# sosp2021/Reth

Measured on AMD Instinct MI355X. Metric: env-steps/sec + learner updates/sec, Ape-X DQN Pong, 1/2/4/8 MI355X, higher is better.
Workload: dtype f32

## Files before the change

include/reth_hip.h:

```cpp
#ifndef RETH_HIP_H
#define RETH_HIP_H
#include <stdint.h>

#ifdef __cplusplus
extern "C" {
#endif

#define RTH_OK 0
#define RTH_ERR_INVALID -1
#define RTH_ERR_HIP -2
#define RTH_ERR_NOMEM -3

#define RTH_U8 0
#define RTH_I32 1
#define RTH_I64 2
#define RTH_F32 3
#define RTH_F64 4
#define RTH_MAX_COLS 8
#define RTH_PRIO_RAW 16
#define RTH_FRAMES 8

const char *rth_last_error(void);
int rth_tree_update_timeouts(int64_t *out);
int rth_version(void);
// ... 182 lines not shown
                       const float *td_abs_dev, float *td_acc_dev, void *stream);
int rth_td_heads_backward(const float *q_s0_dev, const float *q_s1_online_dev, const float *q_s1_target_dev,
                          const int64_t *a_dev, const float *r_dev, const float *done_dev, const double *isw_dev,
                          int64_t B, int64_t A, float gamma_n, int32_t double_q, const float *h_dev, int64_t ldh,
                          const float *w2_dev, int32_t H2, float *td_abs_dev, float *loss_out_dev, float *gh_dev,
                          float *gw2_dev, float *gb2_dev, float *gb1_dev, float *td_acc_dev, void *stream);
int rth_heads_backward_branches(const float *dq_dev, const float *h_dev, int64_t ldh, const float *const *fc2_params_dev,
                                int32_t H, int64_t B, int64_t A, float *gh_dev, float *const *fc2_grads_dev,
                                float *gb1_dev, const float *td_abs_dev, float *td_acc_dev, void *stream);
int rth_td_heads_backward_branches(const float *q_s0_dev, const float *q_s1_online_dev, const float *q_s1_target_dev,
                                   const int64_t *a_dev, const float *r_dev, const float *done_dev,
                                   const double *isw_dev, int64_t B, int64_t A, float gamma_n, int32_t double_q,
                                   const float *h_dev, int64_t ldh, const float *const *fc2_params_dev, int32_t H,
                                   float *td_abs_dev, float *loss_out_dev, float *gh_dev,
                                   float *const *fc2_grads_dev, float *gb1_dev, float *td_acc_dev, void *stream);
int rth_heads_fc2(const float *h_dev, int64_t ldh, int64_t n, int32_t H, int32_t A, const float *const *fc2_params_dev,
                  float *heads_dev, void *stream);
int rth_heads_fc2_upto(const float *h_dev, int64_t ldh, int64_t n_max, const int64_t *n_dev, int32_t H, int32_t A,
                       const float *const *fc2_params_dev, float *heads_dev, float *cache_dev,
                       const int64_t *cache_rows_dev, void *stream);
int rth_linear_relu_rows_upto(const float *x_dev, int64_t ldx, int64_t r0, int64_t n_max, const int64_t *n_dev,
                              const float *w_dev, const float *b_dev, int64_t F, int64_t O, float *y_dev, int64_t ldy,
                              void *stream);

#define RTH_CONV_F32_NHWC 0
#define RTH_CONV_U8_CHW 1
#define RTH_CONV_OUT_NCHW 16
#define RTH_CONV_PACK_DGRAD 32
typedef struct rth_conv_shape {
  int32_t input;
  int32_t cin, hin, win, cout, kh, kw, stride;
} rth_conv_shape;
int rth_conv_supported(const rth_conv_shape *shape);
#define RTH_CONV_IMPL_F32 1
#define RTH_CONV_IMPL_BF16X3 2
#define RTH_CONV_IMPL_X9 3
int rth_conv_impl(const rth_conv_shape *shape, int64_t n, int32_t *nsamp_out);
int64_t rth_conv_packed_bytes(const rth_conv_shape *shape);
int rth_conv_pack(const rth_conv_shape *shape, const float *w_ohwi_dev, float *packed_dev, void *stream);
int rth_conv_pack_many(int32_t n, const rth_conv_shape *shapes, const float *const *w_ohwi_dev,
                       float *const *packed_dev, void *stream);
int rth_conv_bias_relu(const rth_conv_shape *shape, const void *x_dev, const int64_t *rows_dev, int64_t n,
                       const float *packed_dev, const float *bias_dev, float *y_dev, void *stream);
int rth_conv_bias_relu_upto(const rth_conv_shape *shape, const void *x_dev, const int64_t *rows_dev, int64_t n_max,
                            const int64_t *n_dev, const float *packed_dev, const float *bias_dev, float *y_dev,
                            void *stream);
int rth_conv_dgrad_supported(const rth_conv_shape *shape);
int rth_conv_dgrad(const rth_conv_shape *shape, const float *gy_dev, int64_t n, const float *w_ohwi_dev,
                   float *gx_dev, void *stream);
int64_t rth_conv_dgrad_workspace(const rth_conv_shape *shape);
int rth_conv_dgrad_prepacked(const rth_conv_shape *shape, const float *gy_dev, int64_t n, const void *packed_dev,
                             float *gx_dev, void *stream);
int rth_conv_dgrad_relu_supported(const rth_conv_shape *shape);
int rth_conv_dgrad_relu_prepacked(const rth_conv_shape *shape, const float *gy_dev, int64_t n, const void *packed_dev,
                                  const float *y_dev, float *gx_dev, void *bias_ws_dev, int64_t *slabs_out,
                                  void *stream);
int rth_conv_dgrad_relu_nchw_supported(const rth_conv_shape *shape);
int rth_conv_dgrad_relu_nchw_prepacked(const rth_conv_shape *shape, const float *g_dev, const float *y_dev, int64_t n,
                                       const void *packed_dev, const float *y_below_dev, float *gy_dev, float *gx_dev,
                                       void *bias_ws_dev, void *bias_ws_below_dev, int64_t *slabs_out, void *stream);
int rth_fc_x9_supported(int64_t M, int64_t N, int64_t K);
int64_t rth_fc_x9_workspace(int64_t M, int64_t N, int64_t K);
int rth_fc_x9(const float *x_dev, int64_t ldx, int64_t M, const float *w_dev, int64_t N, int64_t K,
              const float *bias_dev, int32_t relu, float *y_dev, void *workspace_dev, void *stream);
int rth_fc_x9_rows_upto(const float *x_dev, int64_t ldx, int64_t M, int64_t n_max, const int64_t *n_dev,
                        const float *w_dev, int64_t N, int64_t K, const float *bias_dev, float *y_dev,
                        void *workspace_dev, void *stream);
int rth_fc1_heads_supported(int64_t M, int64_t N, int64_t K, int32_t A);
int rth_fc1_heads(const float *x_dev, int64_t ldx, int64_t M, const float *w1_dev, int64_t N, int64_t K,
                  const float *b1_dev, int32_t A, const float *const *fc2_params, float *heads_dev, float *h1_out_dev,
                  void *workspace_dev, void *stream);
int rth_fc_f32_supported(int64_t M, int64_t N, int64_t K);
int64_t rth_fc_f32_workspace(int64_t M, int64_t N, int64_t K);
int rth_fc_f32(const float *x_dev, int64_t ldx, int64_t M, const float *w_dev, int64_t N, int64_t K,
               const float *bias_dev, int32_t relu, float *y_dev, void *workspace_dev, void *stream);
int rth_fc_bwd_supported(int64_t B, int64_t N, int64_t K);
int64_t rth_fc_bwd_workspace(int64_t B, int64_t N, int64_t K);
int rth_fc_bwd(const float *gy_dev, int64_t ldg, const float *x_dev, int64_t ldx, const float *w_dev, int64_t B,
               int64_t N, int64_t K, float *gx_dev, float *gw_dev, void *workspace_dev, void *stream);
int rth_conv_dgrad_ws(const rth_conv_shape *shape, const float *gy_dev, int64_t n, const float *w_ohwi_dev,
                      float *gx_dev, void *workspace_dev, void *stream);
int rth_conv_wgrad_x9_supported(const rth_conv_shape *shape);
int64_t rth_conv_wgrad_x9_workspace(const rth_conv_shape *shape);
int rth_conv_wgrad_x9(const rth_conv_shape *shape, const float *x_dev, int64_t n, const float *gy_dev, float *gw_dev,
                      void *workspace_dev, void *stream);
int rth_conv_wgrad_f32_supported(const rth_conv_shape *shape);
int64_t rth_conv_wgrad_f32_workspace(const rth_conv_shape *shape);
int rth_conv_wgrad_f32(const rth_conv_shape *shape, const float *x_dev, int64_t n, const float *gy_dev, float *gw_dev,
                       void *workspace_dev, void *stream);
typedef struct rth_wgrad_deferred {
  const float *partial;
  float *gw;
  int32_t splits, elems, nb, K;
} rth_wgrad_deferred;
int rth_conv_wgrad_f32_partials(const rth_conv_shape *shape, const float *x_dev, int64_t n, const float *gy_dev,
                                float *gw_dev, void *workspace_dev, rth_wgrad_deferred *job_out, void *stream);
int64_t rth_conv_wgrad_workspace(const rth_conv_shape *shape);
int rth_conv_relu_wgrad(const rth_conv_shape *shape, const void *x_dev, const int64_t *rows_dev, int64_t n,
                        const float *g_dev, const float *y_dev, float *gw_dev, float *gb_dev, void *workspace_dev,
                        void *stream);
typedef struct rth_bias_deferred {
  const void *workspace;
  float *db;
  int64_t rows;
  int32_t C;
  int32_t slabs;
} rth_bias_deferred;
int rth_conv_relu_wgrad_ex(const rth_conv_shape *shape, const void *x_dev, const int64_t *rows_dev, int64_t n,
                           const float *g_dev, const float *y_dev, float *gw_dev, float *gb_dev, void *workspace_dev,
                           const rth_bias_deferred *deferred, int32_t ndeferred,
                           const rth_wgrad_deferred *wdeferred, int32_t nwdeferred, void *stream);
int rth_conv1_frames_bias_relu(const rth_conv_shape *shape, const uint8_t *store_dev, const int32_t *ids_dev,
                               int64_t n, const float *packed_dev, const float *bias_dev, float *y_dev, void *stream);
int rth_conv1_frames_relu_wgrad_ex(const rth_conv_shape *shape, const uint8_t *store_dev, const int32_t *ids_dev,
                                   int64_t n, const float *g_dev, const float *y_dev, float *gw_dev, float *gb_dev,
                                   void *workspace_dev, const rth_bias_deferred *deferred, int32_t ndeferred,
                                   const rth_wgrad_deferred *wdeferred, int32_t nwdeferred, void *stream);

typedef struct rth_atari rth_atari;
int rth_atari_create(int32_t in_h, int32_t in_w, int32_t out_h, int32_t out_w, int device, rth_atari **out);
int rth_atari_destroy(rth_atari *h);
int rth_atari_step(rth_atari *h, const uint8_t *raw_dev, int64_t n, uint8_t *frames_dev, int32_t ring, int32_t stack,
                   const int64_t *prev_slot_dev, const int64_t *new_slot_dev, const uint8_t *reset_dev,
                   uint8_t *out_frame_dev, void *stream);
int rth_atari_env_step(rth_atari *h, const uint8_t *raw_dev, int64_t n, uint8_t *frames_dev, int32_t ring,
                       int32_t stack, const int64_t *s0_h_dev, const int64_t *s1_h_dev, const float *done_dev,
                       const int64_t *cur_slot_dev, const uint8_t *reset_raw_dev, void *stream);
int rth_atari_synth_raw(uint8_t *raw_dev, int64_t nbytes, uint64_t seed, const int64_t *t_dev, void *stream);
int rth_atari_synth_reset(uint8_t *reset_raw_dev, int64_t n, int64_t frame_bytes, uint64_t seed, const int64_t *t_dev,
                          const float *done_dev, void *stream);

#define RTH_MAX_PARAM_TENSORS 32
typedef struct rth_param_tensor {
  float *param;
  const float *grad;
  float *exp_avg;
  float *exp_avg_sq;
  int64_t n;
} rth_param_tensor;
int64_t rth_clip_adam_workspace(void);
int rth_clip_adam(const rth_param_tensor *tensors, int32_t n_tensors, double lr, double beta1, double beta2,
                  double eps, double max_norm, int64_t *step_dev, void *workspace_dev, float *total_norm_out_dev,
                  void *stream);
int rth_conv1_relu_wgrad_norm(const rth_conv_shape *shape, const void *x_dev, const int64_t *rows_dev,
                              const int32_t *fids_dev, int64_t n, const float *g_dev, const float *y_dev,
                              float *gw_dev, float *gb_dev, void *workspace_dev, const rth_bias_deferred *deferred,
                              int32_t ndeferred, const rth_wgrad_deferred *wdeferred, int32_t nwdeferred,
                              const rth_param_tensor *sq, int32_t n_sq, double lr, double beta1,
                              double beta2, int64_t *step_dev, void *adam_workspace_dev, int32_t *nparts_out,
                              void *stream);
int rth_adam_prenormed(const rth_param_tensor *tensors, int32_t n_tensors, double lr, double beta1, double beta2,
                       double eps, double max_norm, int32_t nparts, int64_t *step_dev, void *workspace_dev,
                       float *total_norm_out_dev, void *stream);

int rth_mlp_supported(int64_t D, int64_t H, int64_t A);
int64_t rth_mlp_workspace(int64_t B, int64_t D, int64_t H, int64_t A);
int rth_mlp_q(const float *const *params, const float *x_dev, int64_t ldx, int64_t n, int64_t D, int64_t H, int64_t A,
              float *q_dev, int32_t *argmax_dev, void *stream);
int rth_mlp_dqn_grads(const float *const *online, const float *const *target, const float *s0_dev, int64_t lds0,
                      const float *s1_dev, int64_t lds1, const int64_t *a_dev, const float *r_dev,
                      const float *done_dev, const double *isw_dev, int64_t B, int64_t D, int64_t H, int64_t A,
                      float gamma_n, int32_t double_q, float *const *grads, float *td_abs_dev, float *loss_dev,
                      void *workspace_dev, void *stream);

typedef struct rth_mlp_actor_args {
  const float *const *params;
  int64_t D, H, A;
  double *state;
  int32_t *ep_steps;
  int64_t *t_dev;
  int64_t *stats;
  float *obs_ring;
  int64_t *cur_slot;
  const double *eps;
  const int64_t *action_in;
  int64_t *action;
  float *reward, *done;
  int64_t *s0_h, *s1_h;
  int32_t *emit;
  int64_t *row_s0, *row_a, *row_s1;
  float *row_r, *row_done;
  float *row_obs0, *row_obs1;
  float *q_out;
  uint64_t seed;
  int64_t N;
  int32_t ring;
  int32_t max_episode_steps;
} rth_mlp_actor_args;
int rth_cartpole_reset(const rth_mlp_actor_args *args, void *stream);
int rth_mlp_actor_step(rth_nstep *h, const rth_mlp_actor_args *args, void *stream);

enum { RTH_ENV_CARTPOLE = 0, RTH_ENV_ACROBOT = 1, RTH_ENV_MOUNTAINCAR = 2 };
typedef struct rth_env_actor_args {
  const float *const *params;
  int64_t env;
  int64_t D, H, A;
  double *state;
  int32_t *ep_steps;
  int64_t *t_dev;
  int64_t *stats;
  double *ret_stats;
  float *obs_ring;
  int64_t *cur_slot;
  const double *eps;
  const int64_t *action_in;
  int64_t *action;
  float *reward, *done;
  int64_t *s0_h, *s1_h;
  int32_t *emit;
  int64_t *row_s0, *row_a, *row_s1;
  float *row_r, *row_done;
  float *row_obs0, *row_obs1;
  float *q_out;
  uint64_t seed;
  int64_t N;
  int32_t ring;
  int32_t max_episode_steps;
} rth_env_actor_args;
int rth_env_reset(const rth_env_actor_args *args, void *stream);
int rth_env_actor_step(rth_nstep *h, const rth_env_actor_args *args, void *stream);

int rth_ddpg_supported(int64_t D, int64_t Ad, int64_t H1, int64_t H2);
int64_t rth_ddpg_workspace(int64_t B, int64_t D, int64_t Ad, int64_t H1, int64_t H2);
int rth_ddpg_act(const float *const *actor, const float *x_dev, int64_t ldx, int64_t n, int64_t D, int64_t Ad,
                 int64_t H1, int64_t H2, float *act_out_dev, void *stream);
int rth_ddpg_critic_grads(const float *const *critic, const float *const *actor_target,
                          const float *const *critic_target, const float *s0_dev, int64_t lds0, const float *a_dev,
                          int64_t lda, const float *r_dev, const float *done_dev, const float *s1_dev, int64_t lds1,
                          const float *isw_dev, int64_t B, int64_t D, int64_t Ad, int64_t H1, int64_t H2, float gamma,
                          float *const *grads, float *td_abs_dev, float *loss_dev, void *workspace_dev, void *stream);
int rth_ddpg_actor_grads(const float *const *actor, const float *const *critic, const float *s0_dev, int64_t lds0,
                         int64_t B, int64_t D, int64_t Ad, int64_t H1, int64_t H2, float *const *grads,
                         float *loss_dev, void *workspace_dev, void *stream);
int rth_soft_update(float *const *target, const float *const *source, const int64_t *numel, int32_t n_tensors,
                    double tau, void *stream);

int rth_ppo_supported(int64_t D, int64_t H, int64_t A);
int64_t rth_ppo_workspace(int64_t B, int64_t D, int64_t H, int64_t A);
int rth_ppo_act(const float *const *actor, const float *x_dev, int64_t ldx, int64_t n, int64_t D, int64_t H, int64_t A,
                const double *uniforms_dev, uint64_t seed, uint64_t counter, int64_t *action_dev, float *logprob_dev,
                float *probs_dev, void *stream);
int rth_ppo_grads(const float *const *actor, const float *const *value, const float *s_dev, int64_t lds,
                  const int64_t *a_dev, const float *ret_dev, const float *old_logprob_dev, int64_t B, int64_t D,
                  int64_t H, int64_t A, float eps_clip, float vf_coef, float ent_coef, float *const *actor_grads,
                  float *const *value_grads, float *loss_abs_dev, float *loss_mean_dev, void *workspace_dev,
                  void *stream);
int rth_ppo_grads_n(const float *const *actor, const float *const *value, const float *s_dev, int64_t lds,
                    const int64_t *a_dev, const float *ret_dev, const float *old_logprob_dev, int64_t B, int64_t D,
                    int64_t H, int64_t A, float eps_clip, float vf_coef, float ent_coef, float *const *actor_grads,
                    float *const *value_grads, float *loss_abs_dev, float *loss_mean_dev, void *workspace_dev,
                    const int64_t *n_dev, void *stream);
int rth_ppo_grads_adv(const float *const *actor, const float *const *value, const float *s_dev, int64_t lds,
                      const int64_t *a_dev, const float *ret_dev, const float *adv_dev, const float *old_logprob_dev,
                      int64_t B, int64_t D, int64_t H, int64_t A, float eps_clip, float vf_coef, float ent_coef,
                      float *const *actor_grads, float *const *value_grads, float *loss_abs_dev, float *loss_mean_dev,
                      void *workspace_dev, const int64_t *n_dev, void *stream);
int rth_ppo_adv_normalize(float *adv_dev, int64_t B, const int64_t *n_dev, void *stream);
int64_t rth_ppo_shuffle_workspace(int64_t B);
int rth_ppo_shuffle(const float *s_dev, int64_t lds, const int64_t *a_dev, const float *ret_dev, const float *adv_dev,
                    const float *old_logprob_dev, int64_t B, const int64_t *n_dev, int64_t D, int64_t K, uint64_t seed,
                    int64_t *counter_dev, const uint64_t *keys_in, float *mb_s_dev, int64_t *mb_a_dev,
                    float *mb_ret_dev, float *mb_adv_dev, float *mb_logprob_dev, int64_t *mb_n_dev, int32_t *perm_dev,
                    void *workspace_dev, void *stream);

typedef struct rth_ppo_actor_args {
  const float *const *actor;
  int64_t env;
  int64_t D, H, A;
  double *state;
  int32_t *ep_steps;
  int64_t *t_dev;
  int64_t *stats;
  double *ret_stats;
  float *cur_obs;
  const int64_t *action_in;
  const double *uniforms_in;
  int64_t *action;
  float *logprob;
  float *seg_s;
  int64_t *seg_a;
  float *seg_r, *seg_done, *seg_logp;
  int32_t *fill;
  int32_t *complete;
  int32_t *gen;
  int64_t *dropped;
  uint64_t seed;
  int64_t N;
  int32_t cap;
  int32_t max_episode_steps;
} rth_ppo_actor_args;
int rth_ppo_env_reset(const rth_ppo_actor_args *args, void *stream);
int rth_ppo_actor_step(const rth_ppo_actor_args *args, void *stream);
int rth_ppo_rollout_finish(const rth_ppo_actor_args *args, double gamma, float *batch_s_dev, int64_t *batch_a_dev,
                           float *batch_ret_dev, float *batch_logprob_dev, int64_t *n_dev, void *stream);
int rth_ppo_gae_finish(const rth_ppo_actor_args *args, const float *const *value, double gamma, double lam,
                       float *batch_s_dev, int64_t *batch_a_dev, float *batch_ret_dev, float *batch_adv_dev,
                       float *batch_v_dev, float *batch_logprob_dev, int64_t *n_dev, void *stream);
int rth_ppo_actor_step_tl(const rth_ppo_actor_args *args, float *seg_trunc_dev, float *seg_term_s_dev, void *stream);
int rth_ppo_gae_finish_tl(const rth_ppo_actor_args *args, const float *const *value, double gamma, double lam,
                          float *batch_s_dev, int64_t *batch_a_dev, float *batch_ret_dev, float *batch_adv_dev,
                          float *batch_v_dev, float *batch_logprob_dev, int64_t *n_dev, const float *seg_trunc_dev,
                          const float *seg_term_s_dev, void *stream);

enum { RTH_DDPG_ENV_PENDULUM = 0 };
typedef struct rth_ddpg_actor_args {
  const float *const *actor;
// ... 46 lines not shown
```

reth_amd/_lib.py:

```python
import ctypes
import os

_HERE = os.path.dirname(os.path.abspath(__file__))
LIB_PATH = os.environ.get("RTH_LIB_PATH") or os.path.join(_HERE, "libreth_hip.so")

RTH_U8, RTH_I32, RTH_I64, RTH_F32, RTH_F64 = 0, 1, 2, 3, 4
RTH_PRIO_RAW = 16
RTH_FRAMES = 8
SAMPLER_PER, SAMPLER_UNIFORM, SAMPLER_FIFO = 0, 1, 2
MAX_COLS = 8

c_i32, c_i64, c_u64, c_f32, c_f64, c_vp = (ctypes.c_int32, ctypes.c_int64, ctypes.c_uint64,
                                          ctypes.c_float, ctypes.c_double, ctypes.c_void_p)


class HipExtensionMissing(ImportError):
    pass


class RethHipError(RuntimeError):
    pass


class ColDesc(ctypes.Structure):
# ... 79 lines not shown
                ("cap", c_i32), ("max_episode_steps", c_i32)]


DDPG_ENV_PENDULUM = 0


class DdpgActorArgs(ctypes.Structure):
    _fields_ = [("actor", ctypes.POINTER(c_vp)), ("env", c_i64), ("D", c_i64), ("Ad", c_i64), ("H1", c_i64),
                ("H2", c_i64), ("state", c_vp), ("ep_steps", c_vp), ("t_dev", c_vp), ("stats", c_vp),
                ("ret_stats", c_vp), ("noise", c_vp), ("cur_obs", c_vp), ("action_in", c_vp), ("act_det", c_vp),
                ("row_s0", c_vp), ("row_a", c_vp), ("row_r", c_vp), ("row_s1", c_vp), ("row_done", c_vp),
                ("seed", c_u64), ("N", c_i64), ("mu", c_f64), ("theta", c_f64), ("sigma", c_f64),
                ("eps_start", c_f64), ("eps_end", c_f64), ("eps_steps", c_i64), ("max_episode_steps", c_i32),
                ("reserved", c_i32)]


SIGNATURES = {
    "rth_last_error": (ctypes.c_char_p, []),
    "rth_version": (c_i32, []),
    "rth_build_id": (ctypes.c_char_p, []),
    "rth_graph_upload": (c_i32, [c_vp, c_vp]),
    "rth_stream_capture_deps": (c_i32, [c_vp]),
    "rth_sumtree_create": (c_i32, [c_i64, c_i32, ctypes.POINTER(c_vp)]),
    "rth_sumtree_destroy": (c_i32, [c_vp]),
    "rth_sumtree_clear": (c_i32, [c_vp, c_vp]),
    "rth_sumtree_update": (c_i32, [c_vp, c_vp, c_vp, c_i64, c_vp]),
    "rth_sumtree_find": (c_i32, [c_vp, c_vp, c_i64, c_vp, c_vp, c_vp]),
    "rth_sumtree_sample": (c_i32, [c_vp, c_i64, c_vp, c_u64, c_u64, c_vp, c_vp, c_vp]),
    "rth_sumtree_stats": (c_i32, [c_vp, c_vp, c_vp]),
    "rth_sumtree_export": (c_i32, [c_vp, c_vp, c_vp, c_vp, c_vp]),
    "rth_sumtree_import": (c_i32, [c_vp, c_vp, c_vp, c_vp, c_vp]),
    "rth_sumtree_capacity": (c_i64, [c_vp]),
    "rth_per_normalize": (c_i32, [c_vp, c_i64, c_f32, c_vp, c_vp]),
    "rth_per_update": (c_i32, [c_vp, c_vp, c_vp, c_i32, c_i64, c_f64, c_vp]),
    "rth_per_sample": (c_i32, [c_vp, c_i64, c_f64, c_vp, c_u64, c_u64, c_vp, c_vp, c_vp]),
    "rth_replay_create": (c_i32, [c_i64, c_i32, ctypes.POINTER(ColDesc), c_i32, ctypes.POINTER(Sched),
                                  ctypes.POINTER(Sched), c_i32, c_u64, ctypes.POINTER(c_vp)]),
    "rth_replay_destroy": (c_i32, [c_vp]),
    "rth_replay_append": (c_i32, [c_vp, ctypes.POINTER(Src), c_vp, c_i32, c_i64, c_vp, c_vp]),
    "rth_replay_sample": (c_i32, [c_vp, c_i64, c_vp, ctypes.POINTER(c_vp), c_vp, c_vp, c_vp]),
    "rth_replay_update_priorities": (c_i32, [c_vp, c_vp, c_vp, c_i32, c_i64, c_i32, c_vp]),
    "rth_replay_update_priorities_deferred": (c_i32, [c_vp, c_vp, c_vp, c_i32, c_i64, c_i32, c_vp]),
    "rth_replay_flush": (c_i32, [c_vp, c_vp]),
    "rth_replay_gather": (c_i32, [c_vp, c_vp, c_i64, ctypes.POINTER(c_vp), c_vp]),
    "rth_replay_info": (c_i32, [c_vp, ctypes.POINTER(c_i64), ctypes.POINTER(c_i64),
                                ctypes.POINTER(c_i64), ctypes.POINTER(c_i64), ctypes.POINTER(c_i64),
                                ctypes.POINTER(c_i64)]),
    "rth_uniform_indices": (c_i32, [c_i64, c_i64, c_vp, c_u64, c_u64, c_vp, c_vp, c_vp]),
    "rth_replay_tree": (c_vp, [c_vp]),
    "rth_replay_set_timing": (c_i32, [c_vp, ctypes.POINTER(c_vp), c_i32, ctypes.POINTER(c_i32)]),
    "rth_replay_column": (c_vp, [c_vp, c_i32]),
    "rth_replay_frames_attach": (c_i32, [c_vp, c_i64, c_i64, ctypes.POINTER(c_vp), ctypes.POINTER(c_vp)]),
    "rth_replay_push_frames": (c_i32, [c_vp, c_vp, c_i64, c_i32, c_i32, c_vp, c_vp, c_vp, c_vp, c_vp, c_i32, c_vp]),
    "rth_replay_frames_ids_out": (c_i32, [c_vp, c_i32]),
    "rth_copy_rows": (c_i32, [c_vp, c_i64, c_vp, c_vp, c_i64, c_vp, c_i64, c_i64, c_i32, c_i32, c_i32, c_vp]),
    "rth_eps_greedy": (c_i32, [c_vp, c_i64, c_i64, c_i32, c_vp, c_vp, c_vp, c_u64, c_u64, c_vp, c_vp, c_vp]),
    "rth_counter_add": (c_i32, [c_vp, c_i64, c_vp]),
    "rth_actor_prologue": (c_i32, [c_vp, c_vp, c_i64, c_i64, c_vp, c_vp]),
    "rth_compact_flagged": (c_i32, [c_vp, c_vp, c_i64, c_vp, c_i64, c_i64, c_i64, c_vp, c_vp]),
    "rth_actor_tail": (c_i32, [c_vp, ctypes.POINTER(ActorTailArgs), c_vp, c_vp, c_vp, c_vp, c_vp, c_vp, c_vp]),
    "rth_nstep_create": (c_i32, [c_i64, c_i32, c_f64, c_i32, c_i32, ctypes.POINTER(c_vp)]),
    "rth_nstep_destroy": (c_i32, [c_vp]),
    "rth_nstep_reset": (c_i32, [c_vp, c_vp]),
    "rth_nstep_push": (c_i32, [c_vp] + [c_vp] * 11 + [c_vp]),
    "rth_synth_env_step": (c_i32, [c_vp, c_i64, c_i32, c_i64, c_vp, c_vp, c_vp, c_u64, c_f32, c_f32,
                                   c_vp, c_vp, c_vp, c_vp, c_vp]),
    "rth_synth_env_reset": (c_i32, [c_vp, c_i64, c_i32, c_u64, c_vp, c_vp]),
    "rth_game_reset": (c_i32, [ctypes.POINTER(GameArgs), c_vp, c_i64, c_i32, c_vp, c_vp]),
    "rth_game_env_step": (c_i32, [ctypes.POINTER(GameArgs), c_vp, c_i64, c_i32, c_i64, c_vp, c_vp, c_vp, c_vp, c_vp,
                                  c_vp, c_vp, c_vp]),
    "rth_game_actor_tail": (c_i32, [c_vp, ctypes.POINTER(ActorTailArgs), ctypes.POINTER(GameArgs), c_vp, c_vp, c_vp,
                                    c_vp, c_vp, c_vp, c_vp]),
    "rth_td_huber": (c_i32, [c_vp] * 7 + [c_i64, c_i64, c_f32, c_i32, c_i32] + [c_vp] * 5 + [c_vp]),
    "rth_bias_relu": (c_i32, [c_vp, c_vp, c_i64, c_i32, c_vp]),
    "rth_relu_bias_grad_workspace": (c_i64, [c_i32]),
    "rth_heads_merge": (c_i32, [ctypes.POINTER(c_vp), c_i64, c_i64, c_i64, c_i32, c_i32, c_vp, c_vp, c_vp, c_vp,
                                c_vp]),
    "rth_heads_split_grad": (c_i32, [c_vp, c_vp, c_vp, c_vp, c_i64, c_i64, c_i64, c_i32, c_i32,
                                     ctypes.POINTER(c_vp), c_vp]),
    "rth_heads_backward": (c_i32, [c_vp, c_vp, c_i64, c_vp, c_i64, c_i32, c_i32, c_vp, c_vp, c_vp, c_vp, c_vp, c_vp,
                                   c_vp]),
    "rth_td_heads_backward": (c_i32, [c_vp, c_vp, c_vp, c_vp, c_vp, c_vp, c_vp, c_i64, c_i64, c_f32, c_i32, c_vp,
                                      c_i64, c_vp, c_i32, c_vp, c_vp, c_vp, c_vp, c_vp, c_vp, c_vp, c_vp]),
    "rth_heads_backward_branches": (c_i32, [c_vp, c_vp, c_i64, ctypes.POINTER(c_vp), c_i32, c_i64, c_i64, c_vp,
                                            ctypes.POINTER(c_vp), c_vp, c_vp, c_vp, c_vp]),
    "rth_td_heads_backward_branches": (c_i32, [c_vp, c_vp, c_vp, c_vp, c_vp, c_vp, c_vp, c_i64, c_i64, c_f32, c_i32,
                                               c_vp, c_i64, ctypes.POINTER(c_vp), c_i32, c_vp, c_vp, c_vp,
                                               ctypes.POINTER(c_vp), c_vp, c_vp, c_vp]),
    "rth_heads_fc2": (c_i32, [c_vp, c_i64, c_i64, c_i32, c_i32, ctypes.POINTER(c_vp), c_vp, c_vp]),
    "rth_heads_fc2_upto": (c_i32, [c_vp, c_i64, c_i64, c_vp, c_i32, c_i32, ctypes.POINTER(c_vp), c_vp, c_vp, c_vp,
                                   c_vp]),
    "rth_linear_relu_rows_upto": (c_i32, [c_vp, c_i64, c_i64, c_i64, c_vp, c_vp, c_vp, c_i64, c_i64, c_vp, c_i64,
                                          c_vp]),
    "rth_conv_wgrad_x9_supported": (c_i32, [ctypes.POINTER(ConvShape)]),
    "rth_conv_wgrad_x9_workspace": (c_i64, [ctypes.POINTER(ConvShape)]),
    "rth_conv_wgrad_x9": (c_i32, [ctypes.POINTER(ConvShape), c_vp, c_i64, c_vp, c_vp, c_vp, c_vp]),
    "rth_conv_wgrad_f32_supported": (c_i32, [ctypes.POINTER(ConvShape)]),
    "rth_conv_wgrad_f32_workspace": (c_i64, [ctypes.POINTER(ConvShape)]),
    "rth_conv_wgrad_f32": (c_i32, [ctypes.POINTER(ConvShape), c_vp, c_i64, c_vp, c_vp, c_vp, c_vp]),
    "rth_conv_wgrad_f32_partials": (c_i32, [ctypes.POINTER(ConvShape), c_vp, c_i64, c_vp, c_vp, c_vp,
                                            ctypes.POINTER(WgradDeferred), c_vp]),
    "rth_relu_bias_grad": (c_i32, [c_vp, c_vp, c_vp, c_vp, c_vp, c_i64, c_i32, c_vp]),
    "rth_relu_bias_grad_nchw": (c_i32, [c_vp, c_vp, c_vp, c_vp, c_vp, c_i64, c_i32, c_i32, c_vp]),
    "rth_conv_supported": (c_i32, [ctypes.POINTER(ConvShape)]),
    "rth_conv_packed_bytes": (c_i64, [ctypes.POINTER(ConvShape)]),
    "rth_conv_impl": (c_i32, [ctypes.POINTER(ConvShape), c_i64, c_vp]),
    "rth_conv_pack": (c_i32, [ctypes.POINTER(ConvShape), c_vp, c_vp, c_vp]),
    "rth_conv_wgrad_workspace": (c_i64, [ctypes.POINTER(ConvShape)]),
    "rth_conv_relu_wgrad": (c_i32, [ctypes.POINTER(ConvShape), c_vp, c_vp, c_i64, c_vp, c_vp, c_vp, c_vp, c_vp,
                                    c_vp]),
    "rth_conv_relu_wgrad_ex": (c_i32, [ctypes.POINTER(ConvShape), c_vp, c_vp, c_i64, c_vp, c_vp, c_vp, c_vp, c_vp,
                                       c_vp, c_i32, c_vp, c_i32, c_vp]),
    "rth_conv1_frames_relu_wgrad_ex": (c_i32, [ctypes.POINTER(ConvShape), c_vp, c_vp, c_i64, c_vp, c_vp, c_vp, c_vp,
                                               c_vp, c_vp, c_i32, c_vp, c_i32, c_vp]),
    "rth_conv_pack_many": (c_i32, [c_i32, ctypes.POINTER(ConvShape), ctypes.POINTER(c_vp), ctypes.POINTER(c_vp),
                                   c_vp]),
    "rth_conv_bias_relu": (c_i32, [ctypes.POINTER(ConvShape), c_vp, c_vp, c_i64, c_vp, c_vp, c_vp, c_vp]),
    "rth_conv1_frames_bias_relu": (c_i32, [ctypes.POINTER(ConvShape), c_vp, c_vp, c_i64, c_vp, c_vp, c_vp, c_vp]),
    "rth_conv_bias_relu_upto": (c_i32, [ctypes.POINTER(ConvShape), c_vp, c_vp, c_i64, c_vp, c_vp, c_vp, c_vp, c_vp]),
    "rth_conv_dgrad_supported": (c_i32, [ctypes.POINTER(ConvShape)]),
    "rth_conv_dgrad": (c_i32, [ctypes.POINTER(ConvShape), c_vp, c_i64, c_vp, c_vp, c_vp]),
    "rth_conv_dgrad_workspace": (c_i64, [ctypes.POINTER(ConvShape)]),
    "rth_fc_x9_supported": (c_i32, [c_i64, c_i64, c_i64]),
    "rth_fc_x9_workspace": (c_i64, [c_i64, c_i64, c_i64]),
    "rth_fc_x9": (c_i32, [c_vp, c_i64, c_i64, c_vp, c_i64, c_i64, c_vp, c_i32, c_vp, c_vp, c_vp]),
    "rth_fc_x9_rows_upto": (c_i32, [c_vp, c_i64, c_i64, c_i64, c_vp, c_vp, c_i64, c_i64, c_vp, c_vp, c_vp, c_vp]),
    "rth_fc1_heads_supported": (c_i32, [c_i64, c_i64, c_i64, c_i32]),
    "rth_fc1_heads": (c_i32, [c_vp, c_i64, c_i64, c_vp, c_i64, c_i64, c_vp, c_i32, ctypes.POINTER(c_vp), c_vp, c_vp,
                              c_vp, c_vp]),
    "rth_fc_f32_supported": (c_i32, [c_i64, c_i64, c_i64]),
    "rth_fc_f32_workspace": (c_i64, [c_i64, c_i64, c_i64]),
    "rth_fc_f32": (c_i32, [c_vp, c_i64, c_i64, c_vp, c_i64, c_i64, c_vp, c_i32, c_vp, c_vp, c_vp]),
    "rth_fc_bwd_supported": (c_i32, [c_i64, c_i64, c_i64]),
    "rth_fc_bwd_workspace": (c_i64, [c_i64, c_i64, c_i64]),
    "rth_fc_bwd": (c_i32, [c_vp, c_i64, c_vp, c_i64, c_vp, c_i64, c_i64, c_i64, c_vp, c_vp, c_vp, c_vp]),
    "rth_conv_dgrad_ws": (c_i32, [ctypes.POINTER(ConvShape), c_vp, c_i64, c_vp, c_vp, c_vp, c_vp]),
    "rth_conv_dgrad_prepacked": (c_i32, [ctypes.POINTER(ConvShape), c_vp, c_i64, c_vp, c_vp, c_vp]),
    "rth_conv_dgrad_relu_supported": (c_i32, [ctypes.POINTER(ConvShape)]),
    "rth_conv_dgrad_relu_prepacked": (c_i32, [ctypes.POINTER(ConvShape), c_vp, c_i64, c_vp, c_vp, c_vp, c_vp,
                                              ctypes.POINTER(c_i64), c_vp]),
    "rth_conv_dgrad_relu_nchw_supported": (c_i32, [ctypes.POINTER(ConvShape)]),
    "rth_conv_dgrad_relu_nchw_prepacked": (c_i32, [ctypes.POINTER(ConvShape), c_vp, c_vp, c_i64, c_vp, c_vp, c_vp, c_vp,
                                                   c_vp, c_vp, ctypes.POINTER(c_i64), c_vp]),
    "rth_atari_create": (c_i32, [c_i32, c_i32, c_i32, c_i32, c_i32, ctypes.POINTER(c_vp)]),
    "rth_atari_destroy": (c_i32, [c_vp]),
    "rth_atari_step": (c_i32, [c_vp, c_vp, c_i64, c_vp, c_i32, c_i32, c_vp, c_vp, c_vp, c_vp, c_vp]),
    "rth_atari_env_step": (c_i32, [c_vp, c_vp, c_i64, c_vp, c_i32, c_i32, c_vp, c_vp, c_vp, c_vp, c_vp, c_vp]),
    "rth_atari_synth_raw": (c_i32, [c_vp, c_i64, c_u64, c_vp, c_vp]),
    "rth_atari_synth_reset": (c_i32, [c_vp, c_i64, c_i64, c_u64, c_vp, c_vp, c_vp]),
    "rth_clip_adam_workspace": (c_i64, []),
    "rth_tree_update_timeouts": (c_i32, [ctypes.POINTER(c_i64)]),
    "rth_clip_adam": (c_i32, [c_vp, c_i32, c_f64, c_f64, c_f64, c_f64, c_f64, c_vp, c_vp, c_vp, c_vp]),
    "rth_adam_prenormed": (c_i32, [c_vp, c_i32, c_f64, c_f64, c_f64, c_f64, c_f64, c_i32, c_vp, c_vp, c_vp, c_vp]),
    "rth_conv1_relu_wgrad_norm": (c_i32, [ctypes.POINTER(ConvShape), c_vp, c_vp, c_vp, c_i64, c_vp, c_vp, c_vp, c_vp,
                                          c_vp, c_vp, c_i32, c_vp, c_i32, c_vp, c_i32, c_f64, c_f64, c_f64, c_vp, c_vp,
                                          ctypes.POINTER(c_i32), c_vp]),
    "rth_mlp_supported": (c_i32, [c_i64, c_i64, c_i64]),
    "rth_mlp_workspace": (c_i64, [c_i64, c_i64, c_i64, c_i64]),
    "rth_mlp_q": (c_i32, [ctypes.POINTER(c_vp), c_vp, c_i64, c_i64, c_i64, c_i64, c_i64, c_vp, c_vp, c_vp]),
    "rth_mlp_dqn_grads": (c_i32, [ctypes.POINTER(c_vp), ctypes.POINTER(c_vp), c_vp, c_i64, c_vp, c_i64, c_vp, c_vp,
                                  c_vp, c_vp, c_i64, c_i64, c_i64, c_i64, c_f32, c_i32, ctypes.POINTER(c_vp), c_vp,
                                  c_vp, c_vp, c_vp]),
    "rth_ddpg_supported": (c_i32, [c_i64, c_i64, c_i64, c_i64]),
    "rth_ddpg_workspace": (c_i64, [c_i64, c_i64, c_i64, c_i64, c_i64]),
    "rth_ddpg_act": (c_i32, [ctypes.POINTER(c_vp), c_vp, c_i64, c_i64, c_i64, c_i64, c_i64, c_i64, c_vp, c_vp]),
    "rth_ddpg_critic_grads": (c_i32, [ctypes.POINTER(c_vp), ctypes.POINTER(c_vp), ctypes.POINTER(c_vp), c_vp, c_i64,
                                      c_vp, c_i64, c_vp, c_vp, c_vp, c_i64, c_vp, c_i64, c_i64, c_i64, c_i64, c_i64,
                                      c_f32, ctypes.POINTER(c_vp), c_vp, c_vp, c_vp, c_vp]),
    "rth_ddpg_actor_grads": (c_i32, [ctypes.POINTER(c_vp), ctypes.POINTER(c_vp), c_vp, c_i64, c_i64, c_i64, c_i64,
                                     c_i64, c_i64, ctypes.POINTER(c_vp), c_vp, c_vp, c_vp]),
    "rth_soft_update": (c_i32, [ctypes.POINTER(c_vp), ctypes.POINTER(c_vp), ctypes.POINTER(c_i64), c_i32, c_f64,
                                c_vp]),
    "rth_ppo_supported": (c_i32, [c_i64, c_i64, c_i64]),
    "rth_ppo_workspace": (c_i64, [c_i64, c_i64, c_i64, c_i64]),
    "rth_ppo_act": (c_i32, [ctypes.POINTER(c_vp), c_vp, c_i64, c_i64, c_i64, c_i64, c_i64, c_vp, c_u64, c_u64, c_vp,
                            c_vp, c_vp, c_vp]),
    "rth_ppo_grads": (c_i32, [ctypes.POINTER(c_vp), ctypes.POINTER(c_vp), c_vp, c_i64, c_vp, c_vp, c_vp, c_i64, c_i64,
                              c_i64, c_i64, c_f32, c_f32, c_f32, ctypes.POINTER(c_vp), ctypes.POINTER(c_vp), c_vp, c_vp,
                              c_vp, c_vp]),
    "rth_ppo_grads_n": (c_i32, [ctypes.POINTER(c_vp), ctypes.POINTER(c_vp), c_vp, c_i64, c_vp, c_vp, c_vp, c_i64,
                                c_i64, c_i64, c_i64, c_f32, c_f32, c_f32, ctypes.POINTER(c_vp), ctypes.POINTER(c_vp),
                                c_vp, c_vp, c_vp, c_vp, c_vp]),
    "rth_ppo_grads_adv": (c_i32, [ctypes.POINTER(c_vp), ctypes.POINTER(c_vp), c_vp, c_i64, c_vp, c_vp, c_vp, c_vp,
                                  c_i64, c_i64, c_i64, c_i64, c_f32, c_f32, c_f32, ctypes.POINTER(c_vp),
                                  ctypes.POINTER(c_vp), c_vp, c_vp, c_vp, c_vp, c_vp]),
    "rth_ppo_adv_normalize": (c_i32, [c_vp, c_i64, c_vp, c_vp]),
    "rth_ppo_shuffle_workspace": (c_i64, [c_i64]),
    "rth_ppo_shuffle": (c_i32, [c_vp, c_i64, c_vp, c_vp, c_vp, c_vp, c_i64, c_vp, c_i64, c_i64, c_u64, c_vp, c_vp, c_vp,
                                c_vp, c_vp, c_vp, c_vp, c_vp, c_vp, c_vp, c_vp]),
    "rth_ppo_gae_finish": (c_i32, [ctypes.POINTER(PpoActorArgs), ctypes.POINTER(c_vp), c_f64, c_f64, c_vp, c_vp, c_vp,
                                   c_vp, c_vp, c_vp, c_vp, c_vp]),
    "rth_ppo_env_reset": (c_i32, [ctypes.POINTER(PpoActorArgs), c_vp]),
    "rth_ppo_actor_step": (c_i32, [ctypes.POINTER(PpoActorArgs), c_vp]),
    "rth_ppo_actor_step_tl": (c_i32, [ctypes.POINTER(PpoActorArgs), c_vp, c_vp, c_vp]),
    "rth_ppo_gae_finish_tl": (c_i32, [ctypes.POINTER(PpoActorArgs), ctypes.POINTER(c_vp), c_f64, c_f64, c_vp, c_vp, c_vp,
                                      c_vp, c_vp, c_vp, c_vp, c_vp, c_vp, c_vp]),
    "rth_ppo_rollout_finish": (c_i32, [ctypes.POINTER(PpoActorArgs), c_f64, c_vp, c_vp, c_vp, c_vp, c_vp, c_vp]),
    "rth_cartpole_reset": (c_i32, [ctypes.POINTER(MlpActorArgs), c_vp]),
    "rth_mlp_actor_step": (c_i32, [c_vp, ctypes.POINTER(MlpActorArgs), c_vp]),
    "rth_env_reset": (c_i32, [ctypes.POINTER(EnvActorArgs), c_vp]),
    "rth_env_actor_step": (c_i32, [c_vp, ctypes.POINTER(EnvActorArgs), c_vp]),
    "rth_ddpg_env_reset": (c_i32, [ctypes.POINTER(DdpgActorArgs), c_vp]),
    "rth_ddpg_actor_step": (c_i32, [ctypes.POINTER(DdpgActorArgs), c_vp]),
    "rth_weights_create": (c_i32, [c_i64, c_i32, ctypes.POINTER(c_vp)]),
    "rth_weights_destroy": (c_i32, [c_vp]),
    "rth_weights_bytes": (c_i64, [c_vp]),
    "rth_weights_publish": (c_i32, [c_vp, c_i32, ctypes.POINTER(c_vp), ctypes.POINTER(c_i64), c_vp]),
    "rth_weights_fill": (c_i32, [c_vp, c_i32, ctypes.POINTER(c_vp), ctypes.POINTER(c_i64), c_vp]),
    "rth_weights_acquire": (c_i32, [c_vp, c_i32, ctypes.POINTER(c_vp), ctypes.POINTER(c_i64), c_vp, c_vp, c_vp, c_i64,
                                    c_vp, c_vp]),
    "rth_weights_version": (c_i32, [c_vp, ctypes.POINTER(c_i64)]),
    "rth_weights_version_ptr": (c_i32, [c_vp, ctypes.POINTER(c_vp)]),
    "rth_lz4_frame_bound": (c_i32, [c_vp, c_i64, ctypes.POINTER(c_i64)]),
    "rth_lz4_frame_decompress": (c_i32, [c_vp, c_i64, c_vp, c_i64, ctypes.POINTER(c_i64)]),
    "rth_lz4_frame_compress_bound": (c_i64, [c_i64]),
    "rth_lz4_frame_compress": (c_i32, [c_vp, c_i64, c_vp, c_i64, ctypes.POINTER(c_i64)]),
    "rth_xxh32": (ctypes.c_uint32, [c_vp, c_i64, ctypes.c_uint32]),
}

_lib = None
_load_error = None

_SRC_EXT = (".hip", ".hpp", ".cpp", ".h")
HIPCC_FLAGS = ["--offload-arch=gfx950", "-O3", "-fPIC", "-shared", "-std=c++17", "-Wall",
               "-Xclang", "-target-feature", "-Xclang", "-packed-fp32-ops"]


def source_files(root=None):
    root = root or os.path.dirname(_HERE)
    csrc = os.path.join(root, "reth_amd", "csrc")
    rel = sorted(f"reth_amd/csrc/{f}" for f in os.listdir(csrc) if f.endswith(_SRC_EXT))
    return rel + ["include/reth_hip.h"]


def source_build_id(root=None):
    import hashlib

    root = root or os.path.dirname(_HERE)
    h = hashlib.sha1()
    h.update((" ".join(HIPCC_FLAGS) + "\n").encode())
    for rel in source_files(root):
        with open(os.path.join(root, rel), "rb") as f:
            data = f.read()
        blob = hashlib.sha1(b"blob %d\0" % len(data) + data).hexdigest()
        h.update(f"{blob} {rel}\n".encode())
    return h.hexdigest()


def library_build_id(path=None):
    import re

    path = path or LIB_PATH
    try:
        with open(path, "rb") as f:
            m = re.search(rb"RTH_BUILD_ID:([0-9a-f]{40})", f.read())
    except OSError:
        return None
    return m.group(1).decode() if m else None


def _load():
    global _lib, _load_error
    if _lib is not None:
        return _lib
    if not os.path.exists(LIB_PATH):
        _load_error = f"{LIB_PATH} not built (run __graft_entry__.build())"
        raise HipExtensionMissing(_load_error)
    try:
        lib = ctypes.CDLL(LIB_PATH)
    except OSError as e:
        _load_error = str(e)
        raise HipExtensionMissing(f"cannot load {LIB_PATH}: {e}") from e
    for name, (res, args) in SIGNATURES.items():
        fn = getattr(lib, name)
        fn.restype = res
        fn.argtypes = args
    _lib = lib
    return lib


def lib():
    return _load()


def check(rc, what=""):
    if rc != 0:
        msg = _load().rth_last_error().decode(errors="replace")
        raise RethHipError(f"{what or 'libreth_hip'} failed ({rc}): {msg}")


def call(name, *args):
    rc = getattr(_load(), name)(*args)
    check(rc, name)
    return rc


def ptr(t):
    if t is None:
        return None
    return t.data_ptr()


def stream_ptr(stream=None):
    import torch

    s = stream if stream is not None else torch.cuda.current_stream()
# ... 7 lines not shown
```

reth_amd/apex.py:

```python
from dataclasses import dataclass, field
from typing import Optional

import torch

from .actors import OBS_SHAPE, VecActors, apex_columns
from .dist import GradAllReduce
from .model import DQNNetwork
from .replay import HbmReplay
from .reth_buffer import TorchCudaLoader, _SERVICES, start_per
from .solver import Box, DQNSolver, Discrete
from .trainer import Trainer
from .weights import WeightsSlot, WeightsSubscriber

_CAPTURE_MODE = "thread_local"


def _end_part(parts, stream):
    import warnings

    from . import _lib

    empty = _lib.lib().rth_stream_capture_deps(stream.cuda_stream) == 0
    if not empty:
        parts[-1].capture_end()
# ... 113 lines not shown
        return cfg.capacity + reset + (cfg.n_step + 16) * cfg.n_actors + 16

    def close(self):
        _SERVICES.pop(self.addr, None)
        self._graphs = None
        if self.cfg.tuned_gemm:
            from . import gemm_tuning

            gemm_tuning.restore()

    @torch.no_grad()
    def greedy_eval(self, n_envs=256, seed=12345, eps=0.0, action_fn=None):
        cfg = self.cfg
        if cfg.env != "paddle":
            raise RuntimeError("greedy_eval plays the paddle env (ApexConfig.env = 'paddle')")
        torch.cuda.synchronize(self.device)
        net = getattr(self, "_eval_net", None)
        if net is None:
            fmt = torch.channels_last if cfg.channels_last else torch.contiguous_format
            net = self._eval_net = DQNNetwork(OBS_SHAPE, cfg.num_actions).to(self.device, memory_format=fmt)
            net.requires_grad_(False)
            net.hwc_features = bool(cfg.channels_last)
            net.hip_conv = bool(cfg.hip_conv)
        for dst, src in zip(net.parameters(), self.solver.q_network.parameters()):
            dst.copy_(src)
        net.freeze_heads()
        ev = VecActors(n_envs, cfg.num_actions, cfg.n_step, cfg.gamma, self.device, seed=seed, eps=eps,
                       channels_last=cfg.channels_last, env="paddle", balls_per_episode=cfg.balls_per_episode)
        first = torch.zeros(ev.N, dtype=torch.int64, device=self.device)
        got = torch.zeros(ev.N, dtype=torch.bool, device=self.device)
        episodes, _, last, _ = ev.episode_stats()
        for _ in range(38 * cfg.balls_per_episode):
            if action_fn is not None:
                ev.action_in = action_fn(ev)
            ev.step(net)
            new = (episodes > 0) & ~got
            first = torch.where(new, last, first)
            got |= new
        return float((first.sum() / got.sum().clamp(min=1)).item())

    @torch.no_grad()
    def prefill(self, n_rows, chunk=16384):
        g = torch.Generator(device=self.device)
        g.manual_seed(self.cfg.seed + 17 * self.rank)
        done = 0
        if self.replay.frames is not None:
            return self._prefill_frames(n_rows, g, chunk)
        while done < n_rows:
            m = min(chunk, n_rows - done)
            s0 = torch.randint(0, 256, (m, *OBS_SHAPE), dtype=torch.uint8, device=self.device, generator=g)
            s1 = torch.randint(0, 256, (m, *OBS_SHAPE), dtype=torch.uint8, device=self.device, generator=g)
            a = torch.randint(0, self.cfg.num_actions, (m,), dtype=torch.int64, device=self.device, generator=g)
            r = (torch.rand(m, device=self.device, generator=g) < self.cfg.p_reward).float()
            d = (torch.rand(m, device=self.device, generator=g) < self.cfg.p_done).float()
            td = 1.0 - torch.rand(m, device=self.device, generator=g)
            self.replay.append([s0, a, r, s1, d], td)
            done += m

    @torch.no_grad()
    def _prefill_frames(self, n_rows, g, chunk):
        store, K = self.replay.frames, OBS_SHAPE[0]
        F = store.shape[0]
        base = int(self.replay.frame_head)
        nf = n_rows + 2 * K - 1
        if base + nf > F:
            raise ValueError(f"prefill of {n_rows} rows needs {nf} frames behind {base}, the store holds {F}")
        for f0 in range(0, nf, chunk):
            m = min(chunk, nf - f0)
            store[base + f0:base + f0 + m] = torch.randint(0, 256, (m, *store.shape[1:]), dtype=torch.uint8,
                                                           device=self.device, generator=g)
        self.replay.frame_head.fill_(base + nf)
        done = 0
        while done < n_rows:
            m = min(chunk, n_rows - done)
            j = torch.arange(base + done, base + done + m, dtype=torch.int32, device=self.device)[:, None]
            ks = torch.arange(K, dtype=torch.int32, device=self.device)[None, :]
            s0, s1 = (j + ks).contiguous(), (j + K - 1 + ks).contiguous()
            a = torch.randint(0, self.cfg.num_actions, (m,), dtype=torch.int64, device=self.device, generator=g)
            r = (torch.rand(m, device=self.device, generator=g) < self.cfg.p_reward).float()
            d = (torch.rand(m, device=self.device, generator=g) < self.cfg.p_done).float()
            td = 1.0 - torch.rand(m, device=self.device, generator=g)
            self.replay.append([s0, a, r, s1, d], td)
            done += m
        if self.actors.pushes:
            raise RuntimeError("prefill a frame-store replay before the actors step")
        self.actors.attach_frame_store(self.replay)

    def _actor_compute(self):
        if self.cfg.fused_actor:
            return self.actors.step_fused(self.actor_net)
        if self.actors.step(self.actor_net):
            return self.actors.prioritise(self.actor_net), None
        return None, None

    def _learner_train(self, slot):
        data, idx, isw = slot
        return self.trainer.train(data, weights=isw)

    def _actor_host(self):
        if self.subscriber.maybe_load(self.actor_net, self.actors.t):
            self.actors.weights_changed()
            self._ev_acquired = torch.cuda.Event()
            self._ev_acquired.record()

    def _learner_host(self):
        self.trainer.account()
        self.updates += 1
        if self.solver._update_target_interval is not None and not self.solver.auto_target_update:
            self.solver._update_target_interval()
        if self.updates % self.cfg.send_weights_interval == 0:
            if self._ev_acquired is not None:
                torch.cuda.current_stream(self.device).wait_event(self._ev_acquired)
            self.slot.publish(self.solver.q_network)

    def iteration(self):
        if not hasattr(self, "_stream"):
            self._stream = torch.cuda.Stream(self.device, priority=self.cfg.extra.get("actor_priority", 0))
            self._stream.wait_stream(torch.cuda.current_stream(self.device))
        with torch.cuda.stream(self._stream):
            self._iteration()

    def _iteration(self):
        if self._graphs is None and self.cfg.hip_graph and self._graph_ready():
            self._capture()
        if self._graphs is not None:
            return self._iteration_graph()
        for _ in range(self.cfg.actor_steps_per_update):
            self._actor_host()
            td, rows = self._actor_compute()
            if td is not None:
                self.actors.append(self.replay, td, rows)
            self.env_steps += self.actors.N
        if not self.svc.ready():
            return
        if not self.loader.pending():
            self.loader.issue()
        slot = self.loader.take()
        td = self._learner_train(slot)
        self.loader.issue()
        self.replay.update_priorities(slot[1], td, step=True, deferred=True)
        self._learner_host()

    def _graph_ready(self):
        return self.actors.warm and self.updates >= 2 and self.loader.pending() == 1

    def _capture(self):
        solver = self.solver
        solver.auto_target_update = False
        slots = self.loader._slots
        tun = torch.cuda.tunable
        tuning = tun.is_enabled() and tun.tuning_is_enabled()
        if tuning:
            tun.tuning_enable(False)
        try:
            self._capture_graphs(solver, slots)
        finally:
            if tuning:
                tun.tuning_enable(True)

    def _capture_graphs(self, solver, slots):
        host = (self.actors.t, self.actors.pushes)
        side = torch.cuda.Stream(self.device)
        side.wait_stream(torch.cuda.current_stream(self.device))
        split = solver.grad_hook is not None
        G = dict(act=[], act_out=[], tgt=[], q1t=[], learn={}, learn_td={}, buckets={}, grads={})
        psets = [False, True] if self.cfg.extra.get("probe_conv2") else [False]
        with torch.cuda.stream(side):
            act = self.actors
            fresh = act.fresh
            modes = ["full"] + (["dedup"] if self.cfg.fused_actor and self.actor_net.hip_torso else [])
            G["act"], G["act_out"] = {}, {}
            for pr in psets:
                for mode in modes:
                    for _ in range(2):
                        k = act.pushes % 2
                        act.fresh = act.n_step + 2 if mode == "dedup" else 0
                        key = ("probe", mode, k) if pr else (mode, k)
                        if pr and self.cfg.fused_actor:
                            parts, bounds = [torch.cuda.CUDAGraph()], []
                            pool = parts[0]

                            def cut(item, parts=parts, bounds=bounds, pool=pool):
                                _end_part(parts, side)
                                bounds.append(("probe", item))
                                parts.append(torch.cuda.CUDAGraph())
                                parts[-1].capture_begin(pool=pool.pool(), capture_error_mode=_CAPTURE_MODE)

                            parts[0].capture_begin(capture_error_mode=_CAPTURE_MODE)
                            out = act.step_fused(self.actor_net, dedup=mode == "dedup", probe=cut)
                            _end_part(parts, side)
                            G["act"][key] = (parts, bounds)
                        else:
                            g = torch.cuda.CUDAGraph()
                            with torch.cuda.graph(g, stream=side, capture_error_mode=_CAPTURE_MODE):
                                out = (act.step_fused(self.actor_net, dedup=mode == "dedup") if self.cfg.fused_actor
                                       else self._actor_compute())
                            G["act"][key] = g
                        G["act_out"][key] = out
            act.fresh = fresh
            side_tgt = torch.cuda.Stream(self.device)
            side_tgt.wait_stream(side)
            for p in range(2):
                g = torch.cuda.CUDAGraph()
                with torch.cuda.graph(g, stream=side_tgt, capture_error_mode=_CAPTURE_MODE):
                    q1t = solver.target_heads(slots[p][0][3])
                G["tgt"].append(g)
                G["q1t"].append(q1t)
            side.wait_stream(side_tgt)
            for pr, variant, p in [(pr, variant, p) for pr in psets for variant in ("full", "pre") for p in range(2)]:
                    v = ("probe", variant, p) if pr else (variant, p)
                    parts, bounds = [torch.cuda.CUDAGraph()], []
                    pool = parts[0]

                    ended = []

                    def cut(item, last=False, parts=parts, bounds=bounds, ended=ended, pool=pool):
                        _end_part(parts, side)
                        bounds.append(item)
                        if last:
                            ended.append(True)
                            return
                        parts.append(torch.cuda.CUDAGraph())
                        parts[-1].capture_begin(pool=pool.pool(), capture_error_mode=_CAPTURE_MODE)

                    parts[0].capture_begin(capture_error_mode=_CAPTURE_MODE)
                    data, idx, isw = slots[p]
                    probe = (lambda items, last=False: cut(("probe", items), last=last)) if pr else None
                    td = solver.compute_grads(data, isw, q1t=G["q1t"][p] if variant == "pre" else None,
                                              mid=(lambda b: cut(("bucket", b))) if split else None, probe=probe,
                                              prenorm=not split)
                    self.trainer._track(td)
                    if split and not any(k == "bucket" for k, _ in bounds):
                        cut(("bucket", [q.grad for q in solver._params]))
                    solver.apply_grads(probe=probe)
                    if not ended:
                        _end_part(parts, side)
                    G["learn"][v], G["buckets"][v], G["learn_td"][v] = parts, bounds, td
                    G["grads"][v] = [q.grad for q in solver._params]
        torch.cuda.current_stream(self.device).wait_stream(side)
        self.actors.t, self.actors.pushes = host
        self._graphs = G

    def _iteration_graph(self):
        if self.cfg.overlap:
            return self._iteration_graph_overlap()
        G = self._graphs
        act = self.actors
        self._actor_block_graph()
        k = self.loader._pending.pop(0)
        v = self._learner_key(("full", k))
        self._learner_replay(v)
        self.loader.issue()
        self.replay.update_priorities(self.loader._slots[k][1], G["learn_td"][v], step=True, deferred=True)
        self._learner_host()

    def upload_graphs(self):
        from . import _lib

        G = self._graphs
        if G is None:
            return 0
        graphs = list(G["tgt"])
        for g in G["act"].values():
            graphs += g[0] if isinstance(g, tuple) else [g]
        for parts in G["learn"].values():
            graphs += list(parts)
        graphs = [g for g in graphs if g is not None]
        st = self._stream if hasattr(self, "_stream") else torch.cuda.current_stream(self.device)
        for g in graphs:
            _lib.call("rth_graph_upload", g.raw_cuda_graph_exec(), st.cuda_stream)
        st.synchronize()
        return len(graphs)

    def _probing(self):
        return self.conv_probe is not None and self.cfg.extra.get("probe_conv2")

    def _learner_key(self, v):
        return ("probe", *v) if self._probing() and ("probe", *v) in self._graphs["learn"] else v

    def _replay_parts(self, parts, bounds):
        for i, g in enumerate(parts):
            if g is not None:
                g.replay()
            if i < len(bounds):
                for tag, fn in bounds[i][1]:
                    self.conv_probe(tag)
                    fn()
                    self.conv_probe(tag + "_end")

    def _learner_replay(self, v):
        G = self._graphs
        parts, bounds = G["learn"][v], G["buckets"][v]
        if any(kind == "probe" for kind, _ in bounds):
            for q, g in zip(self.solver._params, G["grads"][v]):
                q.grad = g
        if not bounds:
            if parts[0] is not None:
                parts[0].replay()
            return
        hook = self.solver.grad_hook
        cur = torch.cuda.current_stream(self.device)
        bucket_at = [i for i, (kind, _) in enumerate(bounds) if kind == "bucket"]
        comm = None
        for i, (g, (kind, item)) in enumerate(zip(parts, bounds)):
            if g is not None:
                g.replay()
            if kind == "probe":
                for tag, fn in item:
                    if self.conv_probe is not None:
                        self.conv_probe(tag)
                    fn()
                    if self.conv_probe is not None:
                        self.conv_probe(tag + "_end")
                continue
            key = ("bucket", bucket_at.index(i))
            if i != bucket_at[-1]:
                if comm is None:
                    if not hasattr(self, "_stream_comm"):
                        self._stream_comm = torch.cuda.Stream(self.device)
                    comm = self._stream_comm
                comm.wait_stream(cur)
                with torch.cuda.stream(comm):
                    hook.reduce(item, key=key)
            else:
                hook.reduce(item, key=key)
                if comm is not None:
                    cur.wait_stream(comm)
                    comm = None
        if comm is not None:
            cur.wait_stream(comm)
        if len(parts) > len(bounds) and parts[-1] is not None:
            parts[-1].replay()

    def _actor_block_graph(self):
        G, act = self._graphs, self.actors
        for _ in range(self.cfg.actor_steps_per_update):
            self._actor_host()
            k = act.pushes % 2
            mode = "dedup" if ("dedup", k) in G["act"] and act.dedup_ready(self.actor_net) else "full"
            key = ("probe", mode, k) if self._probing() and ("probe", mode, k) in G["act"] else (mode, k)
            g = G["act"][key]
            if isinstance(g, tuple):
                self._replay_parts(*g)
            else:
                g.replay()
            self.actor_modes[mode] = self.actor_modes.get(mode, 0) + 1
            act.t += 1
            act.pushes += 1
            act.fresh += 1
            td, rows = G["act_out"][key]
            if self.cfg.fused_actor:
                act._bind_rows(act._sets[k])
                if act.pushes - 1 > act.n_step:
                    act.append(self.replay, td, rows)
            else:
                act.append(self.replay, td)
            self.env_steps += act.N

    def actor_iteration(self):
        if self._graphs is None:
            raise RuntimeError("actor_iteration replays the captured actor graphs: run iteration() until captured")
        with torch.cuda.stream(self._stream):
            if hasattr(self, "_ev_learn"):
                self._stream.wait_event(self._ev_learn)
            self._actor_block_graph()

    def _next_learner_variant(self):
        k = self.loader._pending[0]
        ready = getattr(self, "_q1t_ready", None)
        return ("pre" if self.cfg.overlap and ready is not None and ready[k] else "full", k)

    def _iteration_graph_overlap(self):
        G = self._graphs
        A = self._stream
        if not hasattr(self, "_stream_b"):
            self._stream_b = torch.cuda.Stream(self.device, priority=self.cfg.extra.get("learner_priority", 0))
            self._ev_learn = torch.cuda.Event()
            self._ev_sample = torch.cuda.Event()
            self._ev_sample.record(A)
            self._ev_learn.record(A)
            self._q1t_ready = [False, False]
        B = self._stream_b
        A.wait_event(self._ev_learn)
        self._actor_block_graph()
        k = self.loader._pending.pop(0)
        v = self._learner_key(("pre" if self._q1t_ready[k] else "full", k))
        self._q1t_ready[k] = False
        syncs = self.solver._target_syncs
        with torch.cuda.stream(B):
            B.wait_event(self._ev_sample)
            self._learner_replay(v)
            self._learner_host()
            self._ev_learn.record(B)
        self.loader.issue()
        if self.solver._target_syncs == syncs:
            kn = self.loader._pending[-1]
            G["tgt"][kn].replay()
            self._q1t_ready[kn] = True
        self._ev_sample.record(A)
        self.replay.update_priorities(self.loader._slots[k][1], G["learn_td"][v], step=True, deferred=True)
```

reth_amd/csrc/conv.hip:

```cpp
#include <cstdlib>
#include <mutex>
#include <string>

#include "common.hpp"
#include "conv1_u8.hpp"
#include "conv_f32.hpp"
#include "conv_x9.hpp"
#include "optim.hpp"
#include "wgrad.hpp"

namespace rth {

constexpr int kPackMax = 6;
constexpr int kPackDgrad3 = 4, kPackDgrad2 = 5;
struct PackJob {
  int geom[kPackMax];
  const float *w[kPackMax];
  f32x4 *packed[kPackMax];
  int first_block[kPackMax + 1];
  int n;
};

__global__ __launch_bounds__(256) void k_conv_pack_many(PackJob job) {
  int l = 0;
  while (l + 1 < job.n && (int)blockIdx.x >= job.first_block[l + 1]) ++l;
  const int sl = ((int)blockIdx.x - job.first_block[l]) * 256 + threadIdx.x;
  switch (job.geom[l]) {
    case 0: pack_conv1_bf16x3(job.w[l], reinterpret_cast<u32x4 *>(job.packed[l]), sl); break;
    case 1: pack_one<8, 8, 4, 4, 32, 84, 84>(job.w[l], job.packed[l], sl); break;
    case 2: pack_one<4, 4, 2, 32, 64, 20, 20>(job.w[l], job.packed[l], sl); break;
    case kPackDgrad3: pack_dgrad3(job.w[l], reinterpret_cast<u32x4 *>(job.packed[l]), sl); break;
    case kPackDgrad2: pack_dgrad2(job.w[l], reinterpret_cast<u32x4 *>(job.packed[l]), sl); break;
    default: pack_x9<X9_CONV3>(job.w[l], reinterpret_cast<u32x4 *>(job.packed[l]), sl); break;
  }
}

struct ConvLaunch {
  const void *fn, *pack;
  int waves;
  int lds_bytes;
  int per_cu;
  int u8;
  int x9;
  const void *x9fn[5];
  const void *tsfn = nullptr;
  int tsfn_rounds = 0;
};

template <int KH, int KW, int S, int CIN, int HIN, int WIN, int NSAMP, int ROT, int KS>
static ConvLaunch x9_launch() {
  using G = X9Geom<KH, KW, S, CIN, HIN, WIN, NSAMP, ROT, KS>;
  ConvLaunch l{reinterpret_cast<const void *>(&k_conv_x9<KH, KW, S, CIN, HIN, WIN, NSAMP, ROT, KS>),
               reinterpret_cast<const void *>(&k_conv_pack_x9<KH, KW, S, CIN, HIN, WIN, NSAMP, ROT, KS>), 4 * KS,
               G::PACKED_U4 * 16, 1, 0, NSAMP, {}};
  l.x9fn[1] = reinterpret_cast<const void *>(&k_conv_x9<KH, KW, S, CIN, HIN, WIN, 1, ROT, KS>);
  if (NSAMP >= 2) l.x9fn[2] = reinterpret_cast<const void *>(&k_conv_x9<KH, KW, S, CIN, HIN, WIN, (NSAMP >= 2 ? 2 : 1), ROT, KS>);
  if (NSAMP >= 3) l.x9fn[3] = reinterpret_cast<const void *>(&k_conv_x9<KH, KW, S, CIN, HIN, WIN, (NSAMP >= 3 ? 3 : 1), ROT, KS>);
  if (NSAMP >= 4) l.x9fn[4] = reinterpret_cast<const void *>(&k_conv_x9<KH, KW, S, CIN, HIN, WIN, (NSAMP >= 4 ? 4 : 1), ROT, KS>);
  return l;
}

template <int KH, int KW, int S, int CIN, int COUT, int HIN, int WIN, int WAVES, int MB, int TS = 1>
static ConvLaunch conv_launch() {
  static_assert(MB == 1, "conv_bias_relu counts 16-pixel wave tiles");
  using Gm = ConvGeom<KH, KW, S, CIN, COUT, HIN, WIN>;
  ConvLaunch l{reinterpret_cast<const void *>(&k_conv_bias_relu<KH, KW, S, CIN, COUT, HIN, WIN, WAVES, MB, TS>),
               reinterpret_cast<const void *>(&k_conv_pack<KH, KW, S, CIN, COUT, HIN, WIN>), WAVES,
               Gm::LDS_F4 * 16, 0, 0, 0, {}};
  int blocks = 0;
  if (hipOccupancyMaxActiveBlocksPerMultiprocessor(&blocks, l.fn, WAVES * 64, 0) != hipSuccess || blocks < 1)
    blocks = 1;
  l.per_cu = blocks;
  return l;
}

static ConvLaunch conv1_u8_launch() {
  ConvLaunch l{reinterpret_cast<const void *>(&k_conv1_u8_share<false>),
               reinterpret_cast<const void *>(&k_conv1_pack_bf16x3), 4, kC1PackedBytes, 0, 1, 0, {}};
  int blocks = 0;
  if (hipOccupancyMaxActiveBlocksPerMultiprocessor(&blocks, l.fn, 256, 0) != hipSuccess || blocks < 1) blocks = 1;
  l.per_cu = blocks;
  return l;
}

constexpr int kWgPerCu = 2, kX9WgPerCu = 1;

static bool find_conv(const rth_conv_shape &s, ConvLaunch *out, int *geom = nullptr) {
  auto is = [&](int mode, int cin, int hin, int win, int cout, int kh, int kw, int st) {
    return (s.input & ~RTH_CONV_OUT_NCHW) == mode && s.cin == cin && s.hin == hin && s.win == win && s.cout == cout && s.kh == kh &&
           s.kw == kw && s.stride == st;
  };
  if (is(RTH_CONV_U8_CHW, 4, 84, 84, 32, 8, 8, 4)) {
    static const ConvLaunch l = conv1_u8_launch();
    *out = l;
    if (geom) *geom = 0;
  } else if (is(RTH_CONV_F32_NHWC, 4, 84, 84, 32, 8, 8, 4)) {
    static const ConvLaunch l = conv_launch<8, 8, 4, 4, 32, 84, 84, 4, 1>();
    *out = l;
    if (geom) *geom = 1;
  } else if (is(RTH_CONV_F32_NHWC, 32, 20, 20, 64, 4, 4, 2)) {
    static const ConvLaunch l = [] {
      ConvLaunch l = conv_launch<4, 4, 2, 32, 64, 20, 20, 8, 1>();
      l.tsfn = conv_launch<4, 4, 2, 32, 64, 20, 20, 8, 1, 4>().fn;
      l.tsfn_rounds = 4;
      return l;
    }();
    *out = l;
    if (geom) *geom = 2;
  } else if (is(RTH_CONV_F32_NHWC, 64, 9, 9, 64, 3, 3, 1)) {
    static const ConvLaunch l = x9_launch<X9_CONV3>();
    *out = l;
    if (geom) *geom = 3;
  } else {
    return false;
  }
  return true;
}

static int cu_count() {
  static int cus = [] {
    int dev = 0, v = 0;
    if (hipGetDevice(&dev) != hipSuccess || hipDeviceGetAttribute(&v, hipDeviceAttributeMultiprocessorCount, dev) !=
                                                 hipSuccess || v < 1)
      v = 256;
    return v;
  }();
  return cus;
}

}

using namespace rth;

static bool is_dgrad3_x9(const rth_conv_shape *shape) {
  return shape->input == RTH_CONV_F32_NHWC && shape->cin == 64 && shape->hin == 9 && shape->win == 9 &&
         shape->cout == 64 && shape->kh == 3 && shape->kw == 3 && shape->stride == 1;
}
static bool is_dgrad2_x9(const rth_conv_shape *shape) {
  return shape->input == RTH_CONV_F32_NHWC && shape->cin == 32 && shape->hin == 20 &&
         shape->win == 20 && shape->cout == 64 && shape->kh == 4 && shape->kw == 4 && shape->stride == 2;
}

static int dgrad_workspace(u32x4 **ws, size_t bytes, hipStream_t st, u32x4 **out) {
  static std::mutex mu;
  int dev = 0;
  RTH_HIP(hipGetDevice(&dev));
  RTH_REQUIRE(dev >= 0 && dev < 64, "rth_conv_dgrad: device %d out of range", dev);
  std::lock_guard<std::mutex> lock(mu);
  if (!ws[dev]) {
    hipStreamCaptureStatus cs = hipStreamCaptureStatusNone;
    RTH_REQUIRE(hipStreamIsCapturing(st, &cs) == hipSuccess && cs == hipStreamCaptureStatusNone,
                "rth_conv_dgrad: the first data gradient of a geometry on a device must run outside graph capture");
    RTH_HIP(hipMalloc(&ws[dev], bytes));
  }
  *out = ws[dev];
  return RTH_OK;
}

static int64_t dgrad_x9_nsamp(int64_t n, int classes, const void *const *fn, int threads, int cap) {
  int64_t ns = 0;
  double best = 0.0;
  for (int64_t k = 1; k <= 3; ++k) {
    if (!fn[k]) continue;
    int per_cu = 0;
    if (hipOccupancyMaxActiveBlocksPerMultiprocessor(&per_cu, fn[k], threads, 0) != hipSuccess || per_cu < 1)
      per_cu = 1;
    const int64_t slots = (int64_t)cu_count() * (per_cu < cap ? per_cu : cap);
    const int64_t rounds = (classes * ((n + k - 1) / k) + slots - 1) / slots;
    const double cost = (double)rounds * ((double)k + 0.5);
    if (ns == 0 || cost < best) best = cost, ns = k;
  }
  return ns;
}

static int launch_dgrad_x9(const void *fn, const float *gy, int64_t n, int64_t ns, int classes, int threads,
                           const u32x4 *wpk, float *gx, hipStream_t st, const float *ymask = nullptr,
                           float *bpart = nullptr, const float *xmask = nullptr, float *xmasked = nullptr) {
  const int nsi = (int)ns;
  const int64_t grid = (n + ns - 1) / ns;
  const int64_t *n_dev = nullptr;
  const float *bias = nullptr;
  int out_nchw = 0;
  void *args[] = {(void *)&gy,    (void *)&n,     (void *)&n_dev,   (void *)&nsi,    (void *)&wpk,
                  (void *)&bias,  (void *)&gx,    (void *)&out_nchw, (void *)&ymask, (void *)&bpart,
                  (void *)&xmask, (void *)&xmasked};
  RTH_HIP(hipLaunchKernel(fn, dim3((unsigned)grid, (unsigned)classes), dim3(threads), args, 0, st));
  return RTH_OK;
}

enum { kDgrad3Plain = 0, kDgrad3Mask = 1, kDgrad3Nchw = 2 };
static const void *const *dgrad3_table(int mode) {
#define RTH_D3(NS, ...) \
  reinterpret_cast<const void *>(&k_conv_x9<3, 3, 1, 64, 11, 11, NS, 3, kX9Dgrad3KS, 2, ##__VA_ARGS__>)
  static const void *const fn[3][4] = {{nullptr, RTH_D3(1), RTH_D3(2), RTH_D3(3)},
                                       {nullptr, RTH_D3(1, 64, 0, 1), RTH_D3(2, 64, 0, 1), RTH_D3(3, 64, 0, 1)},
                                       {nullptr, RTH_D3(1, 64, 0, 1, 1), RTH_D3(2, 64, 0, 1, 1), nullptr}};
#undef RTH_D3
  return fn[mode];
}
static int64_t dgrad3_nsamp(int64_t n, int mode) {
  return dgrad_x9_nsamp(n, 1, dgrad3_table(mode), X9Dgrad3<1>::NT, kX9WgPerCu);
}
static int conv_dgrad_x9_conv3(const float *gy, int64_t n, const float *w, float *gx, void *user_ws, hipStream_t st,
                               const float *ymask = nullptr, float *bpart = nullptr, const float *xmask = nullptr,
                               float *xmasked = nullptr) {
  static u32x4 *ws[64] = {};
  constexpr int PK = X9Dgrad3<1>::PACKED_U4;
  u32x4 *wpk = static_cast<u32x4 *>(user_ws);
  if (!wpk)
    if (const int rc = dgrad_workspace(ws, (size_t)PK * 16, st, &wpk)) return rc;
  RTH_REQUIRE(n * 49 * 64 * 4 < ((int64_t)1 << 31), "rth_conv_dgrad: gy of %lld samples exceeds 2 GiB", (long long)n);
  if (w) {
    hipLaunchKernelGGL((k_conv_pack_x9_dgrad<3, 3, 64, 64, 11, 11, 1, 3, kX9Dgrad3KS>), dim3((PK + 255) / 256),
                       dim3(256), 0, st, w, wpk);
    RTH_LAUNCHED();
  }
  const int mode = xmask ? kDgrad3Nchw : (ymask ? kDgrad3Mask : kDgrad3Plain);
  const int64_t ns = dgrad3_nsamp(n, mode);
  return launch_dgrad_x9(dgrad3_table(mode)[ns], gy, n, ns, 1, X9Dgrad3<1>::NT, wpk, gx, st, ymask, bpart, xmask,
                         xmasked);
}

static int conv_dgrad_x9_conv2(const float *gy, int64_t n, const float *w, float *gx, void *user_ws, hipStream_t st) {
  static u32x4 *ws[64] = {};
  constexpr int PK = X9Dgrad2<1>::PACKED_U4;
  u32x4 *wpk = static_cast<u32x4 *>(user_ws);
  if (!wpk)
    if (const int rc = dgrad_workspace(ws, (size_t)4 * PK * 16, st, &wpk)) return rc;
  RTH_REQUIRE(n * 400 * 32 * 4 < ((int64_t)1 << 31), "rth_conv_dgrad: gx of %lld samples exceeds 2 GiB", (long long)n);
  if (w) {
    hipLaunchKernelGGL((k_conv_pack_x9_dgrad_cls<32, 64, 1, 3, kX9Dgrad2KS>), dim3((4 * PK + 255) / 256), dim3(256),
                       0, st, w, wpk);
    RTH_LAUNCHED();
  }
  const void *fn[4] = {
      nullptr, reinterpret_cast<const void *>(&k_conv_x9<2, 2, 1, 64, 11, 11, 1, 3, kX9Dgrad2KS, 1, 32, 1>),
      reinterpret_cast<const void *>(&k_conv_x9<2, 2, 1, 64, 11, 11, 2, 3, kX9Dgrad2KS, 1, 32, 1>),
      reinterpret_cast<const void *>(&k_conv_x9<2, 2, 1, 64, 11, 11, 3, 3, kX9Dgrad2KS, 1, 32, 1>)};
  const int64_t ns = dgrad_x9_nsamp(n, 4, fn, X9Dgrad2<1>::NT, 4);
  return launch_dgrad_x9(fn[ns], gy, n, ns, 4, X9Dgrad2<1>::NT, wpk, gx, st);
}

extern "C" {

int rth_conv_supported(const rth_conv_shape *shape) {
  ConvLaunch l;
  if (!shape || !find_conv(*shape, &l)) return 0;
  return (shape->input & RTH_CONV_OUT_NCHW) && l.u8 ? 0 : 1;
}

static int64_t select_launch(const ConvLaunch &l, int64_t n);

int rth_conv_impl(const rth_conv_shape *shape, int64_t n, int32_t *nsamp_out) {
  ConvLaunch l;
  if (nsamp_out) *nsamp_out = 0;
  if (!shape || n < 1 || !find_conv(*shape, &l)) return 0;
  if (nsamp_out) *nsamp_out = (int32_t)select_launch(l, n);
  return l.x9 ? RTH_CONV_IMPL_X9 : (l.u8 ? RTH_CONV_IMPL_BF16X3 : RTH_CONV_IMPL_F32);
}

int64_t rth_conv_packed_bytes(const rth_conv_shape *shape) {
  ConvLaunch l;
  return shape && find_conv(*shape, &l) ? (int64_t)l.lds_bytes : 0;
}

int rth_conv_pack(const rth_conv_shape *shape, const float *w, float *packed, void *stream) {
  RTH_REQUIRE(shape && w && packed, "rth_conv_pack: NULL argument");
  ConvLaunch l;
  RTH_REQUIRE(find_conv(*shape, &l), "rth_conv_pack: geometry not built");
  RTH_REQUIRE(((reinterpret_cast<uintptr_t>(w) | reinterpret_cast<uintptr_t>(packed)) & 15) == 0,
              "rth_conv_pack: misaligned buffer");
  void *args[] = {(void *)&w, (void *)&packed};
  const int slots = l.lds_bytes / 16;
  RTH_HIP(hipLaunchKernel(l.pack, dim3((unsigned)((slots + 255) / 256)), dim3(256), args, 0, as_stream(stream)));
  return RTH_OK;
}

int rth_conv_pack_many(int32_t n, const rth_conv_shape *shapes, const float *const *w, float *const *packed,
                       void *stream) {
  RTH_REQUIRE(n >= 0 && n <= kPackMax && (n == 0 || (shapes && w && packed)), "rth_conv_pack_many: bad arguments");
  PackJob job{};
  job.n = n;
  int blocks = 0;
  for (int l = 0; l < n; ++l) {
    if (shapes[l].input & RTH_CONV_PACK_DGRAD) {
      rth_conv_shape fw = shapes[l];
      fw.input &= ~RTH_CONV_PACK_DGRAD;
      const bool d3 = is_dgrad3_x9(&fw), d2 = is_dgrad2_x9(&fw);
      RTH_REQUIRE(d3 || d2, "rth_conv_pack_many: job %d: no packed data-gradient kernel for this geometry", l);
      RTH_REQUIRE(w[l] && packed[l] && ((reinterpret_cast<uintptr_t>(w[l]) | reinterpret_cast<uintptr_t>(packed[l])) &
                                        15) == 0,
                  "rth_conv_pack_many: layer %d buffer NULL or misaligned", l);
      job.geom[l] = d3 ? kPackDgrad3 : kPackDgrad2;
      job.w[l] = w[l];
      job.packed[l] = reinterpret_cast<f32x4 *>(packed[l]);
      job.first_block[l] = blocks;
      blocks += (int)((rth_conv_dgrad_workspace(&fw) / 16 + 255) / 256);
      continue;
    }
    ConvLaunch cl;
    RTH_REQUIRE(find_conv(shapes[l], &cl, &job.geom[l]), "rth_conv_pack_many: layer %d geometry not built", l);
    RTH_REQUIRE(w[l] && packed[l] && ((reinterpret_cast<uintptr_t>(w[l]) | reinterpret_cast<uintptr_t>(packed[l])) &
                                      15) == 0,
                "rth_conv_pack_many: layer %d buffer NULL or misaligned", l);
    job.w[l] = w[l];
    job.packed[l] = reinterpret_cast<f32x4 *>(packed[l]);
    job.first_block[l] = blocks;
    blocks += (cl.lds_bytes / 16 + 255) / 256;
  }
  job.first_block[n] = blocks;
  if (n == 0) return RTH_OK;
  hipLaunchKernelGGL(k_conv_pack_many, dim3((unsigned)blocks), dim3(256), 0, as_stream(stream), job);
  RTH_LAUNCHED();
  return RTH_OK;
}

static bool is_conv1_u8(const rth_conv_shape *s) {
  return s && s->input == RTH_CONV_U8_CHW && s->cin == 4 && s->hin == 84 && s->win == 84 && s->cout == 32 &&
         s->kh == 8 && s->kw == 8 && s->stride == 4;
}

int64_t rth_conv_wgrad_workspace(const rth_conv_shape *shape) {
  return is_conv1_u8(shape) ? (int64_t)kWgBlocks * (32 * 256 + 32) * 4 : 0;
}

struct NormJob {
  const rth_param_tensor *sq;
  int32_t n_sq;
  double lr, beta1, beta2;
  int64_t *step;
  void *adam_ws;
  int32_t *nparts_out;
};
static int conv1_relu_wgrad(const rth_conv_shape *shape, const void *x, const int64_t *rows, const int32_t *fids,
                            int64_t n, const float *g, const float *y, float *gw, float *gb, void *workspace,
                            const rth_bias_deferred *deferred, int32_t ndeferred, const rth_wgrad_deferred *wdeferred,
                            int32_t nwdeferred, void *stream, const NormJob *norm = nullptr);

int rth_conv_relu_wgrad_ex(const rth_conv_shape *shape, const void *x, const int64_t *rows, int64_t n, const float *g,
                           const float *y, float *gw, float *gb, void *workspace, const rth_bias_deferred *deferred,
                           int32_t ndeferred, const rth_wgrad_deferred *wdeferred, int32_t nwdeferred, void *stream) {
  return conv1_relu_wgrad(shape, x, rows, nullptr, n, g, y, gw, gb, workspace, deferred, ndeferred, wdeferred,
                          nwdeferred, stream);
}

int rth_conv1_frames_relu_wgrad_ex(const rth_conv_shape *shape, const uint8_t *store, const int32_t *ids, int64_t n,
                                   const float *g, const float *y, float *gw, float *gb, void *workspace,
                                   const rth_bias_deferred *deferred, int32_t ndeferred,
                                   const rth_wgrad_deferred *wdeferred, int32_t nwdeferred, void *stream) {
  RTH_REQUIRE(store && ids && (reinterpret_cast<uintptr_t>(ids) & 15) == 0,
              "rth_conv1_frames_relu_wgrad_ex: NULL / misaligned frame store or ids");
  return conv1_relu_wgrad(shape, store, nullptr, ids, n, g, y, gw, gb, workspace, deferred, ndeferred, wdeferred,
                          nwdeferred, stream);
}

int rth_conv1_relu_wgrad_norm(const rth_conv_shape *shape, const void *x, const int64_t *rows, const int32_t *fids,
                              int64_t n, const float *g, const float *y, float *gw, float *gb, void *workspace,
                              const rth_bias_deferred *deferred, int32_t ndeferred, const rth_wgrad_deferred *wdeferred,
                              int32_t nwdeferred, const rth_param_tensor *sq, int32_t n_sq, double lr, double beta1,
                              double beta2, int64_t *step_dev,
                              void *adam_workspace_dev, int32_t *nparts_out, void *stream) {
  RTH_REQUIRE(!(rows && fids) && sq && n_sq >= 1 && n_sq <= RTH_MAX_PARAM_TENSORS && step_dev && adam_workspace_dev &&
                  nparts_out && n > 0,
              "rth_conv1_relu_wgrad_norm: bad arguments (rows and fids, %d tensors, a batch of %lld)", n_sq,
              (long long)n);
  for (int i = 0; i < n_sq; ++i)
    RTH_REQUIRE(sq[i].grad && sq[i].n >= 1, "rth_conv1_relu_wgrad_norm: tensor %d incomplete", i);
  if (fids)
    RTH_REQUIRE((reinterpret_cast<uintptr_t>(fids) & 15) == 0, "rth_conv1_relu_wgrad_norm: misaligned frame ids");
  const NormJob nj{sq, n_sq, lr, beta1, beta2, step_dev, adam_workspace_dev, nparts_out};
  return conv1_relu_wgrad(shape, x, rows, fids, n, g, y, gw, gb, workspace, deferred, ndeferred, wdeferred, nwdeferred,
                          stream, &nj);
}

static int conv1_relu_wgrad(const rth_conv_shape *shape, const void *x, const int64_t *rows, const int32_t *fids,
                            int64_t n, const float *g, const float *y, float *gw, float *gb, void *workspace,
                            const rth_bias_deferred *deferred, int32_t ndeferred, const rth_wgrad_deferred *wdeferred,
                            int32_t nwdeferred, void *stream, const NormJob *norm) {
  RTH_REQUIRE(shape && x && g && y && gw && gb && workspace && n >= 0, "rth_conv_relu_wgrad: NULL argument");
  RTH_REQUIRE(nwdeferred >= 0 && nwdeferred <= kWgradJobsMax && (nwdeferred == 0 || wdeferred),
              "rth_conv_relu_wgrad_ex: %d deferred weight gradients (at most %d)", nwdeferred, kWgradJobsMax);
  WgradJobs wj{};
  wj.n = nwdeferred;
  int wblocks = 0;
  for (int j = 0; j < nwdeferred; ++j) {
    const rth_wgrad_deferred &d = wdeferred[j];
    RTH_REQUIRE(d.gw && (d.splits == 0 || d.partial) && d.splits >= 0 && d.splits <= kWgfRedMax && d.elems > 0 &&
                    d.nb >= 0 && d.K > 0,
                "rth_conv_relu_wgrad_ex: deferred weight gradient %d malformed", j);
    wj.j[j] = WgfJob{d.partial, d.gw, d.splits, d.elems, d.nb, d.K};
    wblocks += wgf_reduce_blocks(wj.j[j]);
  }
  RTH_REQUIRE(ndeferred >= 0 && ndeferred <= kBiasJobsMax && (ndeferred == 0 || deferred),
              "rth_conv_relu_wgrad_ex: %d deferred bias gradients (at most %d)", ndeferred, kBiasJobsMax);
  BiasJobs bj{};
  bj.n = ndeferred;
  for (int j = 0; j < ndeferred; ++j) {
    const rth_bias_deferred &d = deferred[j];
    RTH_REQUIRE(d.workspace && d.db && d.C >= 4 && d.C <= 256 && (d.C & (d.C - 1)) == 0 && d.rows >= 0 &&
                    d.slabs >= 0 && d.slabs <= kBiasSlabs,
                "rth_conv_relu_wgrad_ex: deferred bias gradient %d malformed", j);
    bj.part[j] = static_cast<const float *>(d.workspace);
    bj.db[j] = d.db;
    bj.C[j] = d.C;
    bj.slabs[j] = d.slabs > 0 ? d.slabs : (int)bias_grad_slabs(d.rows, d.C);
  }
  RTH_REQUIRE(is_conv1_u8(shape), "rth_conv_relu_wgrad: only the uint8 conv1 geometry (4x84x84 -> 32, k8 s4) is built");
  float *part = static_cast<float *>(workspace);
  if (n == 0) {
    RTH_HIP(hipMemsetAsync(gw, 0, 32 * 256 * 4, as_stream(stream)));
    RTH_HIP(hipMemsetAsync(gb, 0, 32 * 4, as_stream(stream)));
    for (int j = 0; j < ndeferred; ++j)
      RTH_HIP(hipMemsetAsync(deferred[j].db, 0, deferred[j].C * 4, as_stream(stream)));
    for (int j = 0; j < nwdeferred; ++j)
      RTH_HIP(hipMemsetAsync(wdeferred[j].gw, 0, (size_t)wdeferred[j].elems * 4, as_stream(stream)));
    return RTH_OK;
  }
  hipLaunchKernelGGL(fids ? k_conv1_wgrad_bf16x3<2> : (rows ? k_conv1_wgrad_bf16x3<1> : k_conv1_wgrad_bf16x3<0>),
                     dim3(kWgBlocks), dim3(kWgWaves * 64), 0, as_stream(stream), static_cast<const uint8_t *>(x),
                     fids ? reinterpret_cast<const int64_t *>(fids) : rows, n, g, y, part);
  RTH_LAUNCHED();
  constexpr int RB = (32 * 256 + 32 + 63) / 64;
  if (!norm) {
    hipLaunchKernelGGL((k_wgrad_reduce<8, 8, 4, 32>), dim3(RB + ndeferred + wblocks), dim3(256), 0, as_stream(stream),
                       part, kWgBlocks, gw, gb, bj, wj);
    RTH_LAUNCHED();
    return RTH_OK;
  }
  OptArgs na{};
  const int64_t nsq = opt_segments(norm->sq, norm->n_sq, kOptChunk, &na);
  const int64_t nparts = nsq + RB + ndeferred + wblocks;
  RTH_REQUIRE(nparts <= kMaxPartials, "rth_conv1_relu_wgrad_norm: %lld norm partials (at most %d)",
              (long long)nparts, kMaxPartials);
  auto *npart = static_cast<double *>(norm->adam_ws);
  auto *bc = reinterpret_cast<BiasCorr *>(static_cast<uint8_t *>(norm->adam_ws) + (int64_t)kMaxPartials * 8 + 16);
  const SqStep st{norm->step, bc, norm->lr, norm->beta1, norm->beta2};
  hipLaunchKernelGGL((k_wgrad_reduce_norm<8, 8, 4, 32>), dim3((unsigned)nparts), dim3(256), 0, as_stream(stream), part,
                     kWgBlocks, gw, gb, bj, wj, na, (int)nsq, npart, st, (int)(ndeferred + wblocks));
  RTH_LAUNCHED();
  *norm->nparts_out = (int32_t)nparts;
  return RTH_OK;
}

int rth_conv_relu_wgrad(const rth_conv_shape *shape, const void *x, const int64_t *rows, int64_t n, const float *g,
                        const float *y, float *gw, float *gb, void *workspace, void *stream) {
  return rth_conv_relu_wgrad_ex(shape, x, rows, n, g, y, gw, gb, workspace, nullptr, 0, nullptr, 0, stream);
}

static int64_t select_launch(const ConvLaunch &l, int64_t n) {
  int64_t nsamp = 0;
  const int64_t slots = (int64_t)cu_count() * kX9WgPerCu;
  double best = 0.0;
  for (int64_t s = 1; s <= l.x9; ++s) {
    if (!l.x9fn[s]) continue;
    const int64_t rounds = ((n + s - 1) / s + slots - 1) / slots;
    const double cost = (double)rounds * ((double)s + 0.5);
    if (nsamp == 0 || cost < best) best = cost, nsamp = s;
  }
  return nsamp;
}

static int conv_bias_relu(const rth_conv_shape *shape, const void *x, const int64_t *rows, int64_t n,
                          const int64_t *n_dev, const float *w, const float *bias, float *y, void *stream,
                          const int32_t *fids = nullptr) {
  RTH_REQUIRE(shape && x && w && bias && y && n >= 0, "rth_conv_bias_relu: NULL argument");
  ConvLaunch l;
  RTH_REQUIRE(find_conv(*shape, &l),
              "rth_conv_bias_relu: geometry (input %d, %d x %d x %d -> %d, k %dx%d, stride %d) not built", shape->input,
              shape->cin, shape->hin, shape->win, shape->cout, shape->kh, shape->kw, shape->stride);
// ... 171 lines not shown
```

reth_amd/csrc/optim.hip:

```cpp
#include "optim.hpp"

namespace rth {

struct OptScalars {
  float coef;
  float step_size;
  float bc2_sqrt;
  float total_norm;
};

__device__ OptScalars opt_scalars(double acc, double *red, int clip, float max_norm, BiasCorr bc) {
  const float total = (float)sqrt(block_sum(acc, red));
  float coef = 1.0f;
  if (clip) {
    const float c = max_norm / radd(total, 1e-6f);
    coef = c < 1.0f ? c : 1.0f;
  }
  return OptScalars{coef, bc.step_size, bc.bc2_sqrt, total};
}

struct ScalarArgs {
  int clip;
  float max_norm;
  double lr, beta1, beta2;
  int64_t *step;
  OptScalars *out;
  float *total_out;
  BiasCorr *bc;
};

__global__ __launch_bounds__(kOptThreads) void k_grad_sqsum(OptArgs a, double *__restrict__ part, ScalarArgs sa) {
  grad_sqsum_wg(a, blockIdx.x, part, SqStep{sa.step, sa.bc, sa.lr, sa.beta1, sa.beta2});
}

__global__ __launch_bounds__(kOptThreads) void k_adam(OptArgs a, const double *__restrict__ part, int nparts,
                                                     ScalarArgs sa, float w1, float beta2, float w2, float eps) {
  __shared__ double red[kOptThreads / 64];
  const int64_t b = blockIdx.x;
  const OptSeg &sg = a.seg[seg_of(a, b)];
  const int64_t base = (b - sg.blk0) * kAdamChunk;
  double pacc = 0.0, pl[kPartLoads];
#pragma unroll
  for (int u = 0; u < kPartLoads; ++u) {
    const int k = threadIdx.x + u * kOptThreads;
    pl[u] = part[k < nparts ? k : nparts - 1];
  }
  const BiasCorr bc = *sa.bc;
  auto sum_parts = [&]() __attribute__((always_inline)) {
    __builtin_amdgcn_sched_barrier(0);
#pragma unroll
    for (int u = 0; u < kPartLoads; ++u) asm volatile("" : "+v"(pl[u]));
#pragma unroll
    for (int u = 0; u < kPartLoads; ++u)
      if (threadIdx.x + u * kOptThreads < nparts) pacc = radd(pacc, pl[u]);
    for (int k = threadIdx.x + kPartLoads * kOptThreads; k < nparts; k += kOptThreads) pacc = radd(pacc, part[k]);
  };
  __builtin_amdgcn_sched_barrier(0);
  float4 gv[kAdamV], mv[kAdamV], vv[kAdamV], pv[kAdamV];
  if (sg.vec) {
    const __amdgpu_buffer_rsrc_t rg = seg_rsrc(sg.grad, sg.n), rm = seg_rsrc(sg.m, sg.n), rv = seg_rsrc(sg.v, sg.n),
                                 rp = seg_rsrc(sg.param, sg.n);
#pragma unroll
    for (int k = 0; k < kAdamV; ++k) {
      const int64_t e = base + 4 * (k * kOptThreads + threadIdx.x);
      gv[k] = ld4b(rg, e);
      mv[k] = ld4b(rm, e);
      vv[k] = ld4b(rv, e);
      pv[k] = ld4b(rp, e);
    }
    sum_parts();
  } else {
#pragma unroll
    for (int k = 0; k < kAdamV; ++k) {
      const int64_t e = base + 4 * (k * kOptThreads + threadIdx.x);
      gv[k] = ld4(sg.grad, e, sg.n, 0);
      mv[k] = ld4(sg.m, e, sg.n, 0);
      vv[k] = ld4(sg.v, e, sg.n, 0);
      pv[k] = ld4(sg.param, e, sg.n, 0);
    }
    sum_parts();
  }
  const OptScalars sc = opt_scalars(pacc, red, sa.clip, sa.max_norm, bc);
  if (b == 0 && threadIdx.x == 0) {
    *sa.out = sc;
    if (sa.total_out) *sa.total_out = sc.total_norm;
  }
  const int clip = sa.clip;
  const float coef = sc.coef, step_size = sc.step_size, bc2_sqrt = sc.bc2_sqrt;
  auto adam1 = [&](float g, float &m, float &v, float &p) {
    if (clip) g = rmul(g, coef);
    m = radd(m, rmul(w1, rsub(g, m)));
    v = radd(rmul(v, beta2), rmul(rmul(w2, g), g));
    const float denom = radd(sqrtf(v) / bc2_sqrt, eps);
    p = radd(p, rmul(-step_size, m) / denom);
  };
#pragma unroll
  for (int k = 0; k < kAdamV; ++k) {
    const int64_t e = base + 4 * (k * kOptThreads + threadIdx.x);
    if (e >= sg.n) break;
    adam1(gv[k].x, mv[k].x, vv[k].x, pv[k].x);
    adam1(gv[k].y, mv[k].y, vv[k].y, pv[k].y);
    adam1(gv[k].z, mv[k].z, vv[k].z, pv[k].z);
    adam1(gv[k].w, mv[k].w, vv[k].w, pv[k].w);
    st4(sg.param, e, sg.n, sg.vec, pv[k]);
    st4(sg.m, e, sg.n, sg.vec, mv[k]);
    st4(sg.v, e, sg.n, sg.vec, vv[k]);
  }
}

}

using namespace rth;

extern "C" {

int64_t rth_clip_adam_workspace(void) { return (int64_t)kMaxPartials * 8 + 64; }

constexpr int64_t kMaxTensorElems = (int64_t)1 << 29;

static int adam_launch(const char *who, const rth_param_tensor *tensors, int32_t n_tensors, double lr, double beta1,
                       double beta2, double eps, double max_norm, int64_t *step_dev, void *workspace_dev,
                       float *total_norm_out, int nparts, bool sqsum, hipStream_t s) {
  RTH_REQUIRE(tensors && step_dev && workspace_dev, "%s: NULL argument", who);
  RTH_REQUIRE(n_tensors >= 1 && n_tensors <= RTH_MAX_PARAM_TENSORS, "%s: %d tensors not in [1, %d]", who, n_tensors,
              RTH_MAX_PARAM_TENSORS);
  for (int i = 0; i < n_tensors; ++i) {
    RTH_REQUIRE(tensors[i].param && tensors[i].grad && tensors[i].exp_avg && tensors[i].exp_avg_sq && tensors[i].n >= 1,
                "%s: tensor %d incomplete", who, i);
    RTH_REQUIRE(tensors[i].n < kMaxTensorElems, "%s: tensor %d has %lld elements (fewer than 2^29 = %lld)", who, i,
                (long long)tensors[i].n, (long long)kMaxTensorElems);
  }
  OptArgs a{}, ad{};
  const int64_t blocks = opt_segments(tensors, n_tensors, kOptChunk, &a);
  const int64_t ablocks = opt_segments(tensors, n_tensors, kAdamChunk, &ad);
  if (sqsum) nparts = (int)(blocks < kMaxPartials ? blocks : kMaxPartials + 1);
  RTH_REQUIRE(nparts >= 1 && nparts <= kMaxPartials, "%s: %d norm partials (at most %d)", who, nparts, kMaxPartials);
  auto *part = static_cast<double *>(workspace_dev);
  auto *sc = reinterpret_cast<OptScalars *>(static_cast<uint8_t *>(workspace_dev) + (int64_t)kMaxPartials * 8);
  const int clip = max_norm >= 0.0;
  auto *bcw = reinterpret_cast<BiasCorr *>(static_cast<uint8_t *>(workspace_dev) + (int64_t)kMaxPartials * 8 + 16);
  const ScalarArgs sa{clip, (float)max_norm, lr, beta1, beta2, step_dev, sc, total_norm_out, bcw};
  if (sqsum) {
    hipLaunchKernelGGL(k_grad_sqsum, dim3((unsigned)blocks), dim3(kOptThreads), 0, s, a, part, sa);
    RTH_LAUNCHED();
  }
  hipLaunchKernelGGL(k_adam, dim3((unsigned)ablocks), dim3(kOptThreads), 0, s, ad, part, nparts, sa,
                     (float)(1.0 - beta1), (float)beta2, (float)(1.0 - beta2), (float)eps);
  RTH_LAUNCHED();
  return RTH_OK;
}

int rth_clip_adam(const rth_param_tensor *tensors, int32_t n_tensors, double lr, double beta1, double beta2,
                  double eps, double max_norm, int64_t *step_dev, void *workspace_dev, float *total_norm_out,
                  void *stream) {
  return adam_launch("rth_clip_adam", tensors, n_tensors, lr, beta1, beta2, eps, max_norm, step_dev, workspace_dev,
                     total_norm_out, 0, true, as_stream(stream));
}

int rth_adam_prenormed(const rth_param_tensor *tensors, int32_t n_tensors, double lr, double beta1, double beta2,
                       double eps, double max_norm, int32_t nparts, int64_t *step_dev, void *workspace_dev,
                       float *total_norm_out, void *stream) {
  return adam_launch("rth_adam_prenormed", tensors, n_tensors, lr, beta1, beta2, eps, max_norm, step_dev, workspace_dev,
                     total_norm_out, nparts, false, as_stream(stream));
}

}
```

reth_amd/csrc/optim.hpp:

```cpp
#pragma once

#include "common.hpp"

namespace rth {

constexpr int kOptThreads = 256;
constexpr int kOptChunk = 2048;
constexpr int kAdamChunk = 2048;
#ifndef OPT_PART_LOADS
#define OPT_PART_LOADS 5
#endif
constexpr int kPartLoads = OPT_PART_LOADS;
constexpr int kMaxPartials = 1 << 15;

struct OptSeg {
  float *param;
  const float *grad;
  float *m;
  float *v;
  int64_t n;
  int64_t blk0;
  int vec;
};

constexpr int kOptV = kOptChunk / kOptThreads / 4;
constexpr int kAdamV = kAdamChunk / kOptThreads / 4;

__device__ __forceinline__ double block_sum(double v, double *red4) {
#pragma unroll
  for (int o = 32; o > 0; o >>= 1) v = radd(v, __shfl_down(v, o, 64));
  if ((threadIdx.x & 63) == 0) red4[threadIdx.x >> 6] = v;
  __syncthreads();
  double t = red4[0];
#pragma unroll
  for (int w = 1; w < kOptThreads / 64; ++w) t = radd(t, red4[w]);
  return t;
}

__device__ __forceinline__ float4 ld4(const float *__restrict__ p, int64_t e, int64_t n, int vec) {
  if (vec && e + 3 < n) return *reinterpret_cast<const float4 *>(p + e);
  float4 r = make_float4(0.f, 0.f, 0.f, 0.f);
  if (e < n) r.x = p[e];
  if (e + 1 < n) r.y = p[e + 1];
  if (e + 2 < n) r.z = p[e + 2];
  if (e + 3 < n) r.w = p[e + 3];
  return r;
}

__device__ __forceinline__ __amdgpu_buffer_rsrc_t seg_rsrc(const float *p, int64_t n) {
  const uint64_t a = reinterpret_cast<uint64_t>(p);
  const uint32_t lo = __builtin_amdgcn_readfirstlane((uint32_t)a), hi = __builtin_amdgcn_readfirstlane((uint32_t)(a >> 32));
  const int bytes = __builtin_amdgcn_readfirstlane((int)(n * 4));
  return __builtin_amdgcn_make_buffer_rsrc(reinterpret_cast<void *>(((uint64_t)hi << 32) | lo), 0, bytes, 0x00020000);
}
__device__ __forceinline__ float4 ld4b(__amdgpu_buffer_rsrc_t r, int64_t e) {
  return __builtin_bit_cast(float4, __builtin_amdgcn_raw_buffer_load_b128(r, (uint32_t)(e * 4), 0, 0));
}

__device__ __forceinline__ void st4(float *__restrict__ p, int64_t e, int64_t n, int vec, float4 v) {
  if (vec && e + 3 < n) {
    *reinterpret_cast<float4 *>(p + e) = v;
    return;
  }
  if (e < n) p[e] = v.x;
  if (e + 1 < n) p[e + 1] = v.y;
  if (e + 2 < n) p[e + 2] = v.z;
  if (e + 3 < n) p[e + 3] = v.w;
}

struct OptArgs {
  OptSeg seg[RTH_MAX_PARAM_TENSORS];
  int32_t nseg;
};

__device__ __forceinline__ int seg_of(const OptArgs &a, int64_t b) {
  int s = 0;
  while (s + 1 < a.nseg && b >= a.seg[s + 1].blk0) ++s;
  return s;
}

struct BiasCorr {
  float step_size, bc2_sqrt;
};
__device__ __forceinline__ BiasCorr bias_corr(double lr, double beta1, double beta2, int64_t t) {
  const double bc1 = 1.0 - pow(beta1, (double)t);
  const double bc2 = 1.0 - pow(beta2, (double)t);
  return BiasCorr{(float)(lr / bc1), (float)sqrt(bc2)};
}


struct SqStep {
  int64_t *step;
  BiasCorr *bc;
  double lr, beta1, beta2;
};

__device__ __forceinline__ void grad_sqsum_wg(const OptArgs &a, int64_t b, double *__restrict__ part, SqStep st) {
  __shared__ double red[kOptThreads / 64];
  const OptSeg &sg = a.seg[seg_of(a, b)];
  const int64_t base = (b - sg.blk0) * kOptChunk;
  float4 gv[kOptV];
  if (sg.vec) {
    const __amdgpu_buffer_rsrc_t rg = seg_rsrc(sg.grad, sg.n);
#pragma unroll
    for (int k = 0; k < kOptV; ++k) gv[k] = ld4b(rg, base + 4 * (k * kOptThreads + threadIdx.x));
  } else {
#pragma unroll
    for (int k = 0; k < kOptV; ++k) gv[k] = ld4(sg.grad, base + 4 * (k * kOptThreads + threadIdx.x), sg.n, 0);
  }
  double acc = 0.0;
#pragma unroll
  for (int k = 0; k < kOptV; ++k) {
    const double x = gv[k].x, y = gv[k].y, z = gv[k].z, w = gv[k].w;
    acc = radd(acc, rmul(x, x));
    acc = radd(acc, rmul(y, y));
    acc = radd(acc, rmul(z, z));
    acc = radd(acc, rmul(w, w));
  }
  const double wsum = block_sum(acc, red);
  if (threadIdx.x == 0) {
    part[b] = wsum;
    if (b == 0) {
      const int64_t t = *st.step + 1;
      *st.step = t;
      *st.bc = bias_corr(st.lr, st.beta1, st.beta2, t);
    }
  }
}

inline int64_t opt_segments(const rth_param_tensor *tensors, int n_tensors, int64_t chunk, OptArgs *a) {
  int64_t blocks = 0;
  for (int s = 0; s < n_tensors; ++s) {
    const rth_param_tensor &t = tensors[s];
    const uintptr_t al = reinterpret_cast<uintptr_t>(t.param) | reinterpret_cast<uintptr_t>(t.grad) |
                         reinterpret_cast<uintptr_t>(t.exp_avg) | reinterpret_cast<uintptr_t>(t.exp_avg_sq);
    a->seg[s] = OptSeg{t.param, t.grad, t.exp_avg, t.exp_avg_sq, t.n, blocks, (al & 15) == 0 ? 1 : 0};
    blocks += (t.n + chunk - 1) / chunk;
  }
  a->nseg = n_tensors;
  return blocks;
}

}
```

reth_amd/fused_learner.py:

```python
import os

import torch

from . import _lib
from ._lib import call, ctypes, ptr, stream_ptr
from . import model
from .model import conv_workspace, fc1_relu
from .replay import FrameStacks


TD_HB_MAX = 16384
HIP_DGRAD = {1, 2}
HIP_WGRAD = "f32"
DGRAD_PREPACK = True
DGRAD_MASK = True
DGRAD_NCHW = os.environ.get("RTH_DGRAD_NCHW", "1") != "0"
NORM_IN_BACKWARD = True


def eligible(net, s0, s1):
    if not getattr(net, "hip_torso", False):
        return False
    frames = isinstance(s0, FrameStacks), isinstance(s1, FrameStacks)
    if any(frames):
        return all(frames) and s0.shape == s1.shape and all(
            sh is not None for _, sh in net._torso_shapes(tuple(s0.shape[1:]), True))
    if not (torch.is_tensor(s0) and torch.is_tensor(s1) and s0.is_cuda and s1.is_cuda and s0.dtype == s1.dtype):
        return False
    if s0.dtype not in (torch.uint8, torch.float32) or s0.shape != s1.shape or s0.dim() != 4:
        return False
    shapes = net._torso_shapes(tuple(s0.shape[1:]), s0.dtype == torch.uint8)
    return all(sh is not None for _, sh in shapes)


def _pair(s0, s1):
    u8 = s0.dtype == torch.uint8
    fmt = torch.contiguous_format if u8 else torch.channels_last
    if s0.is_contiguous(memory_format=fmt) and s1.is_contiguous(memory_format=fmt) and s1.stride() == s0.stride() \
            and s1.untyped_storage().data_ptr() == s0.untyped_storage().data_ptr() \
            and s1.data_ptr() == s0.data_ptr() + s0.numel() * s0.element_size():
        return torch.as_strided(s0, (2 * s0.shape[0], *s0.shape[1:]), s0.stride())
    return torch.cat([s0, s1]).contiguous(memory_format=fmt)


def _nhwc(t):
    return t if t.is_contiguous(memory_format=torch.channels_last) else t.contiguous(memory_format=torch.channels_last)


def dueling_grads(solver, s0, a, r, s1, done, isw, q1t=None, td_acc=None, mid=None, probe=None, prenorm=False):
    from .solver import td_huber_forward

    net = solver.q_network
    B = s0.shape[0]
    u8 = s0.dtype == torch.uint8
    frames = isinstance(s0, FrameStacks)
    pair = bool(solver.double_q)
    if frames:
        x = FrameStacks.pair(s0, s1) if pair else s0
    else:
        x = _pair(s0, s1) if pair else (s0 if u8 else _nhwc(s0))
    n = x.shape[0]
    convs = net._convs()
    shapes = [sh for _, sh in net._torso_shapes(tuple(s0.shape[1:]), u8)]
    with torch.no_grad():
        w1, b1, w2, b2 = net._merged_head_weights()
        hp = net._head_params()
        fc2p = net._fc2_ptrs(hp)[0]
        dgp, extra = {}, []
        if DGRAD_PREPACK:
            for li in HIP_DGRAD:
                sh = shapes[li] if li < len(shapes) else None
                if sh is None or _lib.lib().rth_conv_dgrad_workspace(ctypes.byref(sh)) <= 0:
                    continue
                dgp[li] = conv_workspace(net, "dgrad", _lib.lib().rth_conv_dgrad_workspace, sh, x.device)
                flagged = _lib.ConvShape(sh.input | _lib.CONV_PACK_DGRAD, sh.cin, sh.hin, sh.win, sh.cout, sh.kh, sh.kw,
                                         sh.stride)
                extra.append((flagged, _nhwc(convs[li].weight.detach()).data_ptr(), dgp[li].data_ptr()))
        packed = net.pack_convs(u8=u8, extra=extra)
        st = stream_ptr()
        ys, h = [], x
        probed = []
        for li, (conv, shape) in enumerate(zip(convs, shapes)):
            y, launch = net._conv_launch(li, conv, shape, h, packed, li == len(convs) - 1)
            if probe is not None and li in (1, 2):
                probed.append((f"conv{li + 1}", launch))
                if li == min(2, len(convs) - 1):
                    probe(probed)
            else:
                launch()
            ys.append(y)
            h = y
        feat = h.view(n, -1)
        h1 = heads = None
        if w2 is None and model.FC1_HEADS:
            h1 = torch.empty((feat.shape[0], w1.shape[0]), dtype=torch.float32, device=feat.device)
            heads = net._fc1_heads(feat, w1, b1, h1_out=h1)
        if heads is None:
            h1 = fc1_relu(feat, w1, b1, owner=net)
            heads = net._heads_fc2(h1) if w2 is None else torch.addmm(b2, h1, w2.t())
        if q1t is None:
            q1t = solver.target_heads(s1)
        q0 = heads[:B]
        q1o = heads[B:] if pair else None
        H2, A1 = w1.shape[0], hp[4].shape[0] + 1
        Hh = H2 // 2
        gh1 = torch.empty((B, H2), dtype=torch.float32, device=x.device)
        gb1 = torch.empty_like(b1)
        g2 = [torch.empty_like(p) for p in hp[4:]]
        g2p = (_lib.c_vp * 4)(*[t.data_ptr() for t in g2])
        if B * A1 <= TD_HB_MAX:
            dev = x.device
            a = a.to(device=dev, dtype=torch.int64).contiguous().view(-1)
            r = r.to(device=dev, dtype=torch.float32).contiguous().view(-1)
            done = done.to(device=dev, dtype=torch.float32).contiguous().view(-1)
            if isw is not None:
                isw = isw.to(device=dev, dtype=torch.float64).contiguous().view(-1)
            q1t = q1t.contiguous()
            if q1t.shape != q0.shape or a.numel() != B or r.numel() != B or done.numel() != B or \
                    (isw is not None and isw.numel() != B):
                raise ValueError("batch columns / target heads disagree with the batch")
            td_abs = torch.empty(B, dtype=torch.float32, device=dev)
            loss = torch.empty(1, dtype=torch.float32, device=dev)
            def td_launch(q1t=q1t, a=a, r=r, done=done, isw=isw):
                call("rth_td_heads_backward_branches", ptr(q0), ptr(q1o), ptr(q1t), ptr(a), ptr(r), ptr(done), ptr(isw),
                     B, A1 - 1, float(solver.gamma_n), int(bool(solver.double_q)), ptr(h1), h1.stride(0), fc2p, Hh,
                     ptr(td_abs), ptr(loss), ptr(gh1), g2p, ptr(gb1), ptr(td_acc), stream_ptr())

            if probe is not None:
                probe([("td_heads_backward", td_launch)])
            else:
                td_launch()
        else:
            loss, td_abs, dq = td_huber_forward(q0, q1o, q1t, a, r, done, isw, solver.gamma_n, solver.double_q,
                                                want_dq=True, dueling=True)
            call("rth_heads_backward_branches", ptr(dq), ptr(h1), h1.stride(0), fc2p, Hh, B, A1 - 1, ptr(gh1), g2p,
                 ptr(gb1), ptr(td_abs), ptr(td_acc), st)
        hip = model.fc1_backward(gh1, feat[:B], w1, owner=net)
        if hip is not None:
            gfeat, gw1 = hip
        else:
            gfeat = torch.mm(gh1, w1)
            gw1 = torch.mm(gh1.t(), feat[:B])
        if mid is not None:
            mid([gw1, gb1, *g2])
        g = gfeat.view(ys[-1][:B].shape)
        grads = {}
        deferred = []
        wdeferred = []
        rbws = net._relu_bias_ws(convs, x.device)
        fused_below = None
        for li in range(len(convs) - 1, -1, -1):
            conv, y = convs[li], ys[li][:B]
            if li == 0 and u8:
                gw = torch.empty(conv.weight.shape, dtype=torch.float32, device=x.device,
                                 memory_format=torch.channels_last)
                db = torch.empty(conv.out_channels, dtype=torch.float32, device=x.device)
                assert len(deferred) <= 4, "rth_conv_relu_wgrad_ex finishes at most 4 deferred bias gradients"
                jobs = (_lib.BiasDeferred * max(len(deferred), 1))(*deferred)
                wjobs = (_lib.WgradDeferred * max(len(wdeferred), 1))(*wdeferred)
                ws1 = conv_workspace(net, "conv1", _lib.lib().rth_conv_wgrad_workspace, shapes[0], x.device)
                opt = solver.optimizer
                if prenorm and NORM_IN_BACKWARD and mid is None and solver.grad_hook is None and hasattr(opt, "prenorm"):
                    done = {d.db for d in deferred} | {d.gw for d in wdeferred}
                    sq = [gr for gr in [gw1[:Hh], gw1[Hh:], gb1[:Hh], gb1[Hh:], *g2]]
                    sq += [gr for c in convs[1:] for gr in (grads[c.weight], grads[c.bias])
                           if gr.data_ptr() not in done]
                    arr, n_sq = opt.norm_tensors(sq)
                    nparts = ctypes.c_int32(0)
                    call("rth_conv1_relu_wgrad_norm", ctypes.byref(shapes[0]), ptr(x.store) if frames else ptr(x), None,
                         ptr(x.ids) if frames else None, B, ptr(_nhwc(g)), ptr(y), ptr(gw), ptr(db), ptr(ws1), jobs,
                         len(deferred), wjobs, len(wdeferred), arr, n_sq, *opt.prenorm_scalars(),
                         ctypes.byref(nparts), st)
                    opt.prenorm(nparts.value)
                elif frames:
                    call("rth_conv1_frames_relu_wgrad_ex", ctypes.byref(shapes[0]), ptr(x.store), ptr(x.ids), B,
                         ptr(_nhwc(g)), ptr(y), ptr(gw), ptr(db), ptr(ws1), jobs, len(deferred), wjobs,
                         len(wdeferred), st)
                else:
                    call("rth_conv_relu_wgrad_ex", ctypes.byref(shapes[0]), ptr(x), None, B, ptr(_nhwc(g)), ptr(y),
                         ptr(gw), ptr(db), ptr(ws1), jobs, len(deferred), wjobs, len(wdeferred), st)
                grads[conv.weight], grads[conv.bias] = gw, db
                deferred, wdeferred = [], []
                break
            nb, c, hh, ww = y.shape
            defer = u8
            xin = ys[li - 1][:B] if li > 0 else x[:B]
            nchw_fused = li == len(convs) - 1 and li in dgp and li > 0 and defer and DGRAD_MASK and DGRAD_NCHW and \
                li in HIP_DGRAD and fused_below is None and \
                bool(_lib.lib().rth_conv_dgrad_relu_nchw_supported(ctypes.byref(shapes[li])))
            gx = None
            if nchw_fused:
                gy = torch.empty((nb, c, hh, ww), dtype=torch.float32, device=x.device,
                                 memory_format=torch.channels_last)
                db = torch.empty(c, dtype=torch.float32, device=x.device)
                gx = torch.empty(xin.shape, dtype=torch.float32, device=x.device, memory_format=torch.channels_last)
                slabs = ctypes.c_int64(0)
                call("rth_conv_dgrad_relu_nchw_prepacked", ctypes.byref(shapes[li]), ptr(g), ptr(y), B, ptr(dgp[li]),
                     ptr(xin), ptr(gy), ptr(gx), ptr(rbws[li]), ptr(rbws[li - 1]), ctypes.byref(slabs), st)
                deferred.append(_lib.BiasDeferred(rbws[li].data_ptr(), db.data_ptr(), nb * hh * ww, c, 0))
                cb = convs[li - 1].out_channels
                db_below = torch.empty(cb, dtype=torch.float32, device=x.device)
                deferred.append(_lib.BiasDeferred(rbws[li - 1].data_ptr(), db_below.data_ptr(),
                                                  xin.shape[0] * xin.shape[2] * xin.shape[3], cb, slabs.value))
                fused_below = (gx, db_below)
            elif fused_below is not None:
                gy, db = fused_below
                fused_below = None
            else:
                gy = torch.empty((nb, c, hh, ww), dtype=torch.float32, device=x.device,
                                 memory_format=torch.channels_last)
                db = torch.empty(c, dtype=torch.float32, device=x.device)
                if li == len(convs) - 1:
                    call("rth_relu_bias_grad_nchw", ptr(g), ptr(y), ptr(gy), None if defer else ptr(db),
                         ptr(rbws[li]), nb, c, hh * ww, st)
                else:
                    g = _nhwc(g)
                    call("rth_relu_bias_grad", ptr(g), ptr(y), ptr(gy), None if defer else ptr(db), ptr(rbws[li]),
                         nb * hh * ww, c, st)
                if defer:
                    deferred.append(_lib.BiasDeferred(rbws[li].data_ptr(), db.data_ptr(), nb * hh * ww, c, 0))
            w = _nhwc(conv.weight.detach())
            hip_dgrad = not nchw_fused and li in HIP_DGRAD and _lib.lib().rth_conv_dgrad_supported(ctypes.byref(shapes[li]))
            hip_wgrad = bool(HIP_WGRAD) and getattr(_lib.lib(), f"rth_conv_wgrad_{HIP_WGRAD}_supported")(
                ctypes.byref(shapes[li]))
            need = [li > 0 and not hip_dgrad and not nchw_fused, not hip_wgrad, False]
            gw = None
            if need[0] or need[1]:
                gxm, gw, _ = torch.ops.aten.convolution_backward(gy, xin, w, None, list(conv.stride), [0, 0], [1, 1],
                                                                False, [0, 0], 1, need)
                gx = gxm if need[0] else gx
            if hip_wgrad:
# ... 40 lines not shown
```

reth_amd/model.py:

```python

import copy

import torch
from torch import nn

from . import _lib
from ._lib import CONV_OUT_NCHW, ConvShape, c_vp, call, ctypes, lib, ptr, stream_ptr
from .replay import FrameStacks


def conv_out(size, k, s):
    return (size - k) // s + 1


def nchw_out(shape):
    return ConvShape(shape.input | CONV_OUT_NCHW, shape.cin, shape.hin, shape.win, shape.cout, shape.kh, shape.kw,
                     shape.stride)


def workspace(owner, device, kind, key, nbytes, zeroed_u8=False):
    store = owner.__dict__.setdefault("_workspaces", {}) if owner is not None else {}
    key = (device, kind, *key)
    ws = store.get(key)
    if ws is None:
        if callable(nbytes):
            nbytes = nbytes()
        ws = store[key] = torch.zeros(nbytes, dtype=torch.uint8, device=device) if zeroed_u8 else \
            torch.empty(max(nbytes, 16) // 4, dtype=torch.float32, device=device)
    return ws


def conv_workspace(owner, kind, sizer, shape, device):
    return workspace(owner, device, kind, (shape.input, shape.cin, shape.hin, shape.cout),
                     lambda: sizer(ctypes.byref(shape)))


def _copy_without(net, memo, skip):
    new = net.__class__.__new__(net.__class__)
    memo[id(net)] = new
    for k, v in net.__dict__.items():
        if k not in skip:
            new.__dict__[k] = copy.deepcopy(v, memo)
    return new


class DQNNetwork(nn.Module):

    def __init__(self, obs_shape, num_actions, dueling=True, hidden_unit=256):
        super().__init__()
        c, h, w = obs_shape
        self.input_shape, self.num_actions, self.dueling = tuple(obs_shape), num_actions, dueling
        self.features = nn.Sequential(
            nn.Conv2d(c, 32, kernel_size=8, stride=4), nn.ReLU(),
            nn.Conv2d(32, 64, kernel_size=4, stride=2), nn.ReLU(),
            nn.Conv2d(64, 64, kernel_size=3, stride=1), nn.ReLU())
        fh = conv_out(conv_out(conv_out(h, 8, 4), 4, 2), 3, 1)
        fw = conv_out(conv_out(conv_out(w, 8, 4), 4, 2), 3, 1)
        nfeat = 64 * fh * fw
        self._feat_chw = (64, fh, fw)
        self.hwc_features = False
        self.hip_conv = True
        if dueling:
            self.fc_adv = nn.Sequential(nn.Linear(nfeat, hidden_unit), nn.ReLU(), nn.Linear(hidden_unit, num_actions))
            self.fc_value = nn.Sequential(nn.Linear(nfeat, hidden_unit), nn.ReLU(), nn.Linear(hidden_unit, 1))
            self._tie_heads()
        else:
            self.fc = nn.Sequential(nn.Linear(nfeat, 512), nn.ReLU(), nn.Linear(512, num_actions))

    def _tie_heads(self):
        a0, v0 = self.fc_adv[0], self.fc_value[0]
        H = a0.weight.shape[0]
        w = torch.cat([a0.weight.detach(), v0.weight.detach()])
        b = torch.cat([a0.bias.detach(), v0.bias.detach()])
        a0.weight.data, v0.weight.data = w[:H], w[H:]
        a0.bias.data, v0.bias.data = b[:H], b[H:]
        self._w1s, self._b1s = w, b

    def _apply(self, fn, *args, **kwargs):
        out = super()._apply(fn, *args, **kwargs)
        if self.dueling:
            self._tie_heads()
        return out

    def _tie_check(self):
        if not self.dueling:
            return
        a0, v0 = self.fc_adv[0], self.fc_value[0]
        w, b = self.__dict__.get("_w1s"), self.__dict__.get("_b1s")
        H = a0.weight.shape[0]
        ok = (w is not None and b is not None and a0.weight.data_ptr() == w.data_ptr()
              and v0.weight.data_ptr() == w[H:].data_ptr() and a0.bias.data_ptr() == b.data_ptr()
              and v0.bias.data_ptr() == b[H:].data_ptr() and w.device == a0.weight.device)
        if not ok:
            self._tie_heads()

    def __deepcopy__(self, memo):
        new = _copy_without(self, memo, ("_w1s", "_b1s", "_frozen", "_frozen_packed", "_shape_cache", "_workspaces"))
        if new.dueling:
            new._tie_heads()
        return new

    def forward(self, x):
        x = self.features(x).flatten(1)
        if not self.dueling:
            return self.fc(x)
        adv = self.fc_adv(x)
        value = self.fc_value(x)
        return value + adv - adv.mean(dim=1, keepdim=True)

    def _head_params(self):
        a0, v0, a2, v2 = self.fc_adv[0], self.fc_value[0], self.fc_adv[2], self.fc_value[2]
        return [a0.weight, v0.weight, a0.bias, v0.bias, a2.weight, v2.weight, a2.bias, v2.bias]

    def _merged_head_weights(self):
        ps = self._head_params()
        a0, v0, a2, v2 = self.fc_adv[0], self.fc_value[0], self.fc_adv[2], self.fc_value[2]
        A, H = a2.weight.shape
        if torch.is_grad_enabled() and any(p.requires_grad for p in ps):
            if ps[0].is_cuda:
                return _MergeHeads.apply((H, ps[0].shape[1], A, 0, 1), *ps)
            w1, b1 = torch.cat([a0.weight, v0.weight]), torch.cat([a0.bias, v0.bias])
        else:
            self._tie_check()
            w1, b1 = self._w1s, self._b1s
            if ps[0].is_cuda and self._fc2_inplace():
                return w1, b1, None, None
        w2 = torch.cat([torch.cat([a2.weight, a2.weight.new_zeros(A, H)], 1),
                        torch.cat([v2.weight.new_zeros(1, H), v2.weight], 1)])
        b2 = torch.cat([a2.bias, v2.bias])
        return w1, b1, w2, b2

    def _fc2_inplace(self):
        A, H = self.fc_adv[2].weight.shape
        return A <= 32 and H % 64 == 0 and H <= 512

    @property
    def hip_torso(self):
        return bool(self.hwc_features and self.dueling and self.hip_conv)

    def _fc2_ptrs(self, hp=None):
        ps = (hp or self._head_params())[4:]
        return ((c_vp * 4)(*[p.data_ptr() for p in ps]), *ps[0].shape)

    def _heads_fc2(self, h):
        arr, A, H = self._fc2_ptrs()
        out = torch.empty((h.shape[0], A + 1), dtype=torch.float32, device=h.device)
        call("rth_heads_fc2", ptr(h), h.stride(0), h.shape[0], H, A, arr, ptr(out), stream_ptr())
        return out

    def _fc1_heads(self, h, w1, b1, h1_out=None):
        if not (h.is_cuda and h.dim() == 2 and h.stride(1) == 1 and w1.is_contiguous() and self._fc2_inplace()):
            return None
        M, K = h.shape
        N = w1.shape[0]
        arr, A, H = self._fc2_ptrs()
        if N != 2 * H or not lib().rth_fc1_heads_supported(M, N, K, A):
            return None
        out = torch.empty((M, A + 1), dtype=torch.float32, device=h.device)
        ws = _fc_workspace(self, h.device, w1, M, N, K)
        call("rth_fc1_heads", ptr(h), h.stride(0), M, ptr(w1), N, K, ptr(b1), A, arr, ptr(out), ptr(h1_out),
             ptr(ws), stream_ptr())
        return out

    @torch.no_grad()
    def freeze_heads(self):
        self._tie_check()
        merged = list(self._merged_head_weights())
        old = getattr(self, "_frozen", None)
        if old is not None:
            for k in (2, 3):
                if old[k] is not None and merged[k] is not None and old[k].shape == merged[k].shape:
                    old[k].copy_(merged[k])
                    merged[k] = old[k]
        self._frozen = merged
        if self.hwc_features and self._frozen[0].is_cuda:
            self._frozen_packed = self.pack_convs(out=getattr(self, "_frozen_packed", None))

    def forward_heads(self, x, merged=None, rows=None, packed=None, n_dev=None, n_fixed=None, cache=None):
        if not self.dueling:
            raise ValueError("forward_heads needs the dueling network")
        frozen = getattr(self, "_frozen", None) is not None
        if merged is None:
            merged = self._frozen if frozen else self._merged_head_weights()
        w1, b1, w2, b2 = merged
        if self.hwc_features:
            if packed is None and frozen:
                packed = getattr(self, "_frozen_packed", None)
# ... 380 lines not shown
```

reth_amd/optim.py:

```python
import ctypes

import torch

from . import _lib
from ._lib import call, ptr, stream_ptr


class ParamTensor(ctypes.Structure):
    _fields_ = [("param", _lib.c_vp), ("grad", _lib.c_vp), ("exp_avg", _lib.c_vp), ("exp_avg_sq", _lib.c_vp),
                ("n", _lib.c_i64)]


class ClipAdam(torch.optim.Optimizer):
    MAX_TENSORS = 32

    def __init__(self, params, lr=1e-3, betas=(0.9, 0.999), eps=1e-8, max_norm=None):
        super().__init__(params, dict(lr=lr, betas=tuple(betas), eps=eps))
        if len(self.param_groups) != 1:
            raise ValueError("ClipAdam takes one parameter group")
        ps = self.param_groups[0]["params"]
        if not ps or len(ps) > self.MAX_TENSORS:
            raise ValueError(f"ClipAdam: {len(ps)} parameter tensors (1..{self.MAX_TENSORS})")
        dev = ps[0].device
        for p in ps:
            dense = p.is_contiguous() or p.is_contiguous(memory_format=torch.channels_last)
            if p.dtype != torch.float32 or p.device != dev or not dense:
                raise ValueError("ClipAdam: parameters must be dense float32 tensors on one device")
        self.max_norm = max_norm
        self._step = torch.zeros(1, dtype=torch.int64, device=dev)
        self._ws = torch.zeros(_lib.lib().rth_clip_adam_workspace(), dtype=torch.uint8, device=dev)
        self.total_norm = torch.zeros(1, dtype=torch.float32, device=dev)
        self._prenormed = None
        for p in ps:
            st = self.state[p]
            st["exp_avg"] = torch.zeros_like(p)
            st["exp_avg_sq"] = torch.zeros_like(p)
            st["step"] = self._step

    @torch.no_grad()
    def step(self, closure=None, max_norm=None):
        loss = closure() if closure is not None else None
        g = self.param_groups[0]
        beta1, beta2 = g["betas"]
        mn = self.max_norm if max_norm is None else max_norm
        tensors = []
        for p in g["params"]:
            if p.grad is None:
                continue
            gr = p.grad
            if gr.stride() != p.stride():
                gr = torch.empty_like(p).copy_(gr)
            st = self.state[p]
            tensors.append(ParamTensor(p.data_ptr(), gr.data_ptr(), st["exp_avg"].data_ptr(),
                                       st["exp_avg_sq"].data_ptr(), p.numel()))
        if not tensors:
            return loss
        arr = (ParamTensor * len(tensors))(*tensors)
        nparts, self._prenormed = self._prenormed, None
        if nparts is not None:
            call("rth_adam_prenormed", ctypes.cast(arr, _lib.c_vp), len(tensors), float(g["lr"]), float(beta1),
                 float(beta2), float(g["eps"]), -1.0 if mn is None or mn < 0 else float(mn), nparts, ptr(self._step),
                 ptr(self._ws), ptr(self.total_norm), stream_ptr())
            return loss
        call("rth_clip_adam", ctypes.cast(arr, _lib.c_vp), len(tensors), float(g["lr"]), float(beta1), float(beta2),
             float(g["eps"]), -1.0 if mn is None or mn < 0 else float(mn), ptr(self._step), ptr(self._ws),
             ptr(self.total_norm), stream_ptr())
        return loss

    def norm_tensors(self, grads):
        ts = [ParamTensor(gr.data_ptr(), gr.data_ptr(), gr.data_ptr(), gr.data_ptr(), gr.numel()) for gr in grads]
        return (ParamTensor * len(ts))(*ts), len(ts)

    def prenorm_scalars(self):
        g = self.param_groups[0]
        beta1, beta2 = g["betas"]
        return float(g["lr"]), float(beta1), float(beta2), ptr(self._step), ptr(self._ws)

    def step_launch(self, max_norm=None):
        nparts, self._prenormed = self._prenormed, None

        def launch():
            self._prenormed = nparts
            self.step(max_norm=max_norm)

        return launch

    def prenorm(self, nparts):
        self._prenormed = int(nparts)
```

reth_amd/solver.py:

```python
import io

import numpy as np
import torch

from . import _lib, fused_learner
from . import model as _model
from ._lib import call, ptr, stream_ptr
from .model import default_models
from .optim import ClipAdam
from .replay import FrameStacks
from .schedule import Interval


class Discrete:

    def __init__(self, n):
        self.n = int(n)


class Box:

    def __init__(self, low, high, shape, dtype=None):
        self.low, self.high, self.shape = low, high, tuple(shape)

# ... 132 lines not shown
        self.mlp_impl = _model.MLP_IMPL
        self.mlp_hip_launches = 0
        self.mlp_impl_active = "hip" if self.mlp_impl == "hip" and self._mlp_eligible() else None
        if self.mlp_impl_active == "hip":
            self._mlp_grads = [torch.empty_like(p) for p in self.q_network._params6()]
            self._mlp_arrays()

    @torch.no_grad()
    def update_target(self):
        self._target_syncs = getattr(self, "_target_syncs", 0) + 1
        torch._foreach_copy_(self._tparams, self._params)
        if self._heads:
            self.target_q_network.freeze_heads()

    def load_weights(self, stream):
        states = torch.load(stream, map_location=self.device, weights_only=True)
        self.q_network.load_state_dict(states)
        self.update_target()

    def save_weights(self, stream=None):
        if stream is None:
            stream = io.BytesIO()
        torch.save(self.q_network.state_dict(), stream)
        return stream

    def _tensors(self, batch):
        s0, a, r, s1, done = batch
        dev = self.device
        f = lambda x, dt: (x.to(device=dev, dtype=dt, non_blocking=True) if torch.is_tensor(x)
                           else torch.as_tensor(np.asarray(x), dtype=dt).to(dev, non_blocking=True))
        fr = lambda x: x if self._u8_frames(x) else f(x, torch.float32)
        return fr(s0), f(a, torch.int64), f(r, torch.float32), fr(s1), f(done, torch.float32)

    def _u8_frames(self, x):
        return ((torch.is_tensor(x) or isinstance(x, FrameStacks)) and x.dtype == torch.uint8 and x.is_cuda
                and self._heads and getattr(self.q_network, "hip_torso", False))

    def target_heads(self, s1):
        if not self._u8_frames(s1):
            s1 = (s1 if torch.is_tensor(s1) else torch.as_tensor(np.asarray(s1))).to(self.device, torch.float32)
        with torch.no_grad():
            return self.target_q_network.forward_heads(s1) if self._heads else self.target_q_network(s1)

    def _forward_targets(self, s1, merged=None, packed=None, q1t=None):
        with torch.no_grad():
            if self._heads:
                if q1t is None:
                    q1t = self.target_q_network.forward_heads(s1)
                q1o = None
                if self.double_q:
                    m = [t.detach() for t in merged] if merged is not None else None
                    q1o = self.q_network.forward_heads(s1, m, packed=packed)
            else:
                if q1t is None:
                    q1t = self.target_q_network(s1)
                q1o = self.q_network(s1) if self.double_q else None
        return q1o, q1t

    def _mlp_eligible(self):
        q, t = self.q_network, self.target_q_network
        return (type(q) is _model.MLP_DQNNetwork and type(t) is _model.MLP_DQNNetwork and q.dims() == t.dims()
                and q.hip_supported() and t.hip_supported())

    def _mlp_arrays(self):
        key = tuple(p.data_ptr() for p in self.q_network._params6() + self.target_q_network._params6())
        if getattr(self, "_mlp_key", None) != key:
            mk = lambda ts: (_lib.c_vp * 6)(*[t.data_ptr() for t in ts])
            self._mlp_ptrs = (mk(self.q_network._params6()), mk(self.target_q_network._params6()),
                              mk(self._mlp_grads))
            self._mlp_key = key
        return self._mlp_ptrs

    def _mlp_states(self, x):
        D = self.q_network.dims()[0]
        x = (x if torch.is_tensor(x) else torch.as_tensor(np.asarray(x))).to(self.device, torch.float32)
        x = x.reshape(-1, D)
        return x if x.stride(1) == 1 and x.stride(0) >= D else x.contiguous()

    def _mlp_q(self, x):
        D, H, A = self.q_network.dims()
        n = x.shape[0]
        q = torch.empty((n, A), dtype=torch.float32, device=self.device)
        am = torch.empty(n, dtype=torch.int32, device=self.device)
        call("rth_mlp_q", self._mlp_arrays()[0], ptr(x), x.stride(0), n, D, H, A, ptr(q), ptr(am), stream_ptr())
        self.mlp_hip_launches += 1
        return q, am

    def _mlp_td(self, s0, a, r, s1, done, isw, backward):
        D, H, A = self.q_network.dims()
        s0, s1 = self._mlp_states(s0), self._mlp_states(s1)
        B = s0.shape[0]
        a, r, done = a.contiguous().view(-1), r.contiguous().view(-1), done.contiguous().view(-1)
        if isw is not None:
            isw = isw.to(device=self.device, dtype=torch.float64).contiguous().view(-1)
        if s1.shape[0] != B or a.numel() != B or r.numel() != B or done.numel() != B or (
                isw is not None and isw.numel() != B):
            raise ValueError("batch columns disagree in length")
        online, target, grads = self._mlp_arrays()
        td_abs = torch.empty(B, dtype=torch.float32, device=self.device)
        loss = torch.empty(1, dtype=torch.float32, device=self.device)
        ws = self.q_network._mlp_workspace(self.device, B)
        call("rth_mlp_dqn_grads", online, target, ptr(s0), s0.stride(0), ptr(s1), s1.stride(0), ptr(a), ptr(r),
             ptr(done), ptr(isw), B, D, H, A, self.gamma_n, int(bool(self.double_q)), grads if backward else None,
             ptr(td_abs), ptr(loss), ptr(ws), stream_ptr())
        self.mlp_hip_launches += 1
        return loss, td_abs

    def calc_loss_device(self, batch):
        s0, a, r, s1, done = self._tensors(batch)
        if self.mlp_impl_active == "hip":
            return self._mlp_td(s0, a, r, s1, done, None, backward=False)[1]
        with torch.no_grad():
            q0 = self.q_network.forward_heads(s0) if self._heads else self.q_network(s0)
        q1o, q1t = self._forward_targets(s1)
        _, td_abs, _ = td_huber_forward(q0, q1o, q1t, a, r, done, None, self.gamma_n, self.double_q, want_dq=False,
                                        dueling=self._heads)
        return td_abs

    def calc_loss(self, batch):
        return self.calc_loss_device(batch).cpu()

    def compute_grads(self, batch, weights=None, q1t=None, mid=None, probe=None, prenorm=False):
        s0, a, r, s1, done = self._tensors(batch)
        isw = None if weights is None else (weights if torch.is_tensor(weights) else torch.as_tensor(np.asarray(weights)))
        if self.mlp_impl_active == "hip" and q1t is None:
            loss, td_abs = self._mlp_td(s0, a, r, s1, done, isw, backward=True)
            for p, g in zip(self.q_network._params6(), self._mlp_grads):
                p.grad = g
            self.last_loss = loss.view(())
            return td_abs
        if self.fused_grads and self._heads and fused_learner.eligible(self.q_network, s0, s1):
            loss, td_abs = fused_learner.dueling_grads(self, s0, a, r, s1, done, isw, q1t, td_acc=self.td_mean_acc,
                                                        mid=mid, probe=probe, prenorm=prenorm)
            if self.td_mean_acc is not None:
                td_abs._rth_mean_tracked = True
            self.last_loss = loss.detach()
            return td_abs
        merged = packed = None
        if self._heads:
            merged = self.q_network._merged_head_weights()
            if getattr(self.q_network, "hip_torso", False) and merged[0].is_cuda:
                with torch.no_grad():
                    packed = self.q_network.pack_convs()
            q0 = self.q_network.forward_heads(s0, merged, packed=packed)
        else:
            q0 = self.q_network(s0)
        q1o, q1t = self._forward_targets(s1, merged, packed, q1t)
        loss, td_abs = td_huber_loss(q0, q1o, q1t, a, r, done, isw, self.gamma_n, self.double_q, self._heads)
        self.optimizer.zero_grad(set_to_none=True)
        loss.backward()
        self.last_loss = loss.detach()
        return td_abs

    def apply_grads(self, probe=None):
        if isinstance(self.optimizer, ClipAdam):
            if probe is not None:
                tail = self.auto_target_update and self._update_target_interval is not None
                probe([("clip_adam", self.optimizer.step_launch())], last=not tail)
            else:
                self.optimizer.step()
        else:
            if self.clip_value >= 0:
                torch.nn.utils.clip_grad_norm_(self._params, self.clip_value, foreach=True)
            self.optimizer.step()
        if self.auto_target_update and self._update_target_interval is not None:
            self._update_target_interval()

    def update_device(self, batch, weights=None, q1t=None):
        td_abs = self.compute_grads(batch, weights, q1t, prenorm=self.grad_hook is None)
        if self.grad_hook is not None:
            self.grad_hook(self._params)
        self.apply_grads()
        return td_abs

    def update(self, batch, weights=None):
        return self.update_device(batch, weights).cpu()

    @torch.no_grad()
    def act(self, state):
        if self.mlp_impl_active == "hip":
            return int(self._mlp_q(self._mlp_states(state))[1].item())
        x = torch.as_tensor(np.asarray(state), dtype=torch.float32).to(self.device).unsqueeze(0) \
            if not torch.is_tensor(state) else state.to(self.device, torch.float32).unsqueeze(0)
        return int(torch.argmax(self.q_network(x), dim=1).item())

    @torch.no_grad()
    def act_batch(self, states):
        if self.mlp_impl_active == "hip":
            return self._mlp_q(self._mlp_states(states))[1]
        x = (states if torch.is_tensor(states) else torch.as_tensor(np.asarray(states))).to(self.device, torch.float32)
        return torch.argmax(self.q_network(x), dim=1).to(torch.int32)


def get_solver(name, **kwargs):
    if name == "dqn":
        return DQNSolver(**kwargs)
    if name == "ddpg":
        from .ddpg import DDPGSolver

        return DDPGSolver(**kwargs)
    raise NotImplementedError(f"solver {name!r}: only 'dqn' and 'ddpg' are rebuilt")
```

Baseline: 511,100.

## Fuse conv weight repacking into the Adam optimizer step

Adds pack-aware Adam kernels in which blocks that update the conv weight tensors stage the updated weights in shared-memory tiles and write the bf16x3-split packed layouts (forward and dgrad) directly. A version stamp lets the learner skip the separate pack_convs launch on the next forward when the packs are current. This removes one kernel launch and one re-read of the conv weights per learner update, at the cost of a more complex optimizer kernel with tile-shaped work assignment for those tensors and extra staleness bookkeeping.

Measured after the change: 511,500, median of 3. No clear change (+0.1%).

```diff
diff --git a/include/reth_hip.h b/include/reth_hip.h
--- a/include/reth_hip.h
+++ b/include/reth_hip.h
@@ -358,6 +358,14 @@
 int rth_adam_prenormed(const rth_param_tensor *tensors, int32_t n_tensors, double lr, double beta1, double beta2,
                        double eps, double max_norm, int32_t nparts, int64_t *step_dev, void *workspace_dev,
                        float *total_norm_out_dev, void *stream);
+int rth_clip_adam_pack(const rth_param_tensor *tensors, int32_t n_tensors, double lr, double beta1, double beta2,
+                       double eps, double max_norm, int64_t *step_dev, void *workspace_dev,
+                       float *total_norm_out_dev, int32_t n_jobs, const rth_conv_shape *shapes,
+                       const int32_t *job_tensor, float *const *packed_dev, void *stream);
+int rth_adam_prenormed_pack(const rth_param_tensor *tensors, int32_t n_tensors, double lr, double beta1, double beta2,
+                            double eps, double max_norm, int32_t nparts, int64_t *step_dev, void *workspace_dev,
+                            float *total_norm_out_dev, int32_t n_jobs, const rth_conv_shape *shapes,
+                            const int32_t *job_tensor, float *const *packed_dev, void *stream);
 
 int rth_mlp_supported(int64_t D, int64_t H, int64_t A);
 int64_t rth_mlp_workspace(int64_t B, int64_t D, int64_t H, int64_t A);
diff --git a/reth_amd/_lib.py b/reth_amd/_lib.py
--- a/reth_amd/_lib.py
+++ b/reth_amd/_lib.py
@@ -255,6 +255,10 @@
     "rth_tree_update_timeouts": (c_i32, [ctypes.POINTER(c_i64)]),
     "rth_clip_adam": (c_i32, [c_vp, c_i32, c_f64, c_f64, c_f64, c_f64, c_f64, c_vp, c_vp, c_vp, c_vp]),
     "rth_adam_prenormed": (c_i32, [c_vp, c_i32, c_f64, c_f64, c_f64, c_f64, c_f64, c_i32, c_vp, c_vp, c_vp, c_vp]),
+    "rth_clip_adam_pack": (c_i32, [c_vp, c_i32, c_f64, c_f64, c_f64, c_f64, c_f64, c_vp, c_vp, c_vp, c_i32,
+                                   ctypes.POINTER(ConvShape), ctypes.POINTER(c_i32), ctypes.POINTER(c_vp), c_vp]),
+    "rth_adam_prenormed_pack": (c_i32, [c_vp, c_i32, c_f64, c_f64, c_f64, c_f64, c_f64, c_i32, c_vp, c_vp, c_vp, c_i32,
+                                        ctypes.POINTER(ConvShape), ctypes.POINTER(c_i32), ctypes.POINTER(c_vp), c_vp]),
     "rth_conv1_relu_wgrad_norm": (c_i32, [ctypes.POINTER(ConvShape), c_vp, c_vp, c_vp, c_i64, c_vp, c_vp, c_vp, c_vp,
                                           c_vp, c_vp, c_i32, c_vp, c_i32, c_vp, c_i32, c_f64, c_f64, c_f64, c_vp, c_vp,
                                           ctypes.POINTER(c_i32), c_vp]),
diff --git a/reth_amd/apex.py b/reth_amd/apex.py
--- a/reth_amd/apex.py
+++ b/reth_amd/apex.py
@@ -289,6 +289,7 @@
         tuning = tun.is_enabled() and tun.tuning_is_enabled()
         if tuning:
             tun.tuning_enable(False)
+        solver.refresh_learner_packs()
         try:
             self._capture_graphs(solver, slots)
         finally:
@@ -428,6 +429,7 @@
     def _learner_replay(self, v):
         G = self._graphs
         parts, bounds = G["learn"][v], G["buckets"][v]
+        self.solver.refresh_learner_packs()
         if any(kind == "probe" for kind, _ in bounds):
             for q, g in zip(self.solver._params, G["grads"][v]):
                 q.grad = g
diff --git a/reth_amd/csrc/conv.hip b/reth_amd/csrc/conv.hip
--- a/reth_amd/csrc/conv.hip
+++ b/reth_amd/csrc/conv.hip
@@ -32,6 +32,101 @@
     case kPackDgrad3: pack_dgrad3(job.w[l], reinterpret_cast<u32x4 *>(job.packed[l]), sl); break;
     case kPackDgrad2: pack_dgrad2(job.w[l], reinterpret_cast<u32x4 *>(job.packed[l]), sl); break;
     default: pack_x9<X9_CONV3>(job.w[l], reinterpret_cast<u32x4 *>(job.packed[l]), sl); break;
+  }
+}
+
+constexpr int kPackTileCo = 8;
+constexpr int kPackTileMax = kPackTileCo * 192;
+constexpr int kAdamPackSegs = 3;
+struct AdamPackArgs {
+  OptSeg seg[kAdamPackSegs];
+  int K[kAdamPackSegs], L[kAdamPackSegs];
+  int nseg, blocks;
+  int n;
+  int geom[kPackMax], seg_of[kPackMax];
+  u32x4 *packed[kPackMax];
+};
+
+__device__ __forceinline__ u32x4 split_slot(const float (&wv)[8], int t) {
+  uint32_t e[8];
+#pragma unroll
+  for (int j = 0; j < 8; ++j) e[j] = bf16x3_term(wv[j], t);
+  return u32x4{e[0] | (e[1] << 16), e[2] | (e[3] << 16), e[4] | (e[5] << 16), e[6] | (e[7] << 16)};
+}
+
+__device__ __forceinline__ void tile_pack(int geom, int T8, int kp, int i, const float *tile, u32x4 *packed) {
+  float wv[8];
+  switch (geom) {
+    case 0: {
+      if (i >= 384) return;
+      const int r = i & 7, ci = (i >> 3) & 3, khl = (i >> 5) & 3, t = i >> 7;
+      const int rho = ci * 8 + 4 * kp + khl, c = rho >> 1, h = rho & 1;
+#pragma unroll
+      for (int j = 0; j < 8; ++j) wv[j] = tile[r * 128 + khl * 32 + j * 4 + ci];
+      packed[(c * 3 + t) * 64 + h * 32 + T8 * 8 + r] = split_slot(wv, t);
+      return;
+    }
+    case 2: {
+      if (i >= 256) return;
+      const int r = i & 7, f = i >> 3, g = kp * 8 + (f >> 2), q = f & 3, o = T8 * 8 + r;
+      const float4 v = *reinterpret_cast<const float4 *>(tile + r * 128 + 4 * f);
+      reinterpret_cast<f32x4 *>(packed)[(g * 4 + (o >> 4)) * 64 + q * 16 + (o & 15)] = f32x4{v.x, v.y, v.z, v.w};
+      return;
+    }
+    case kPackDgrad2: {
+      if (i >= 384) return;
+      using G = X9Dgrad2<1>;
+      const int ci = i & 31, kw = (i >> 5) & 3, t = i >> 7;
+      const int cls = 2 * (kp & 1) + (kw & 1), tap = 2 * (1 - (kp >> 1)) + (1 - (kw >> 1));
+#pragma unroll
+      for (int j = 0; j < 8; ++j) wv[j] = tile[j * 128 + kw * 32 + ci];
+      packed[cls * G::PACKED_U4 + (((ci >> 4) * G::NCH + tap * 2 + (T8 >> 2)) * 3 + t) * 64 + (T8 & 3) * 16 + (ci & 15)] =
+          split_slot(wv, t);
+      return;
+    }
+    case kPackDgrad3: {
+      if (i >= 576) return;
+      using G = X9Dgrad3<1>;
+      const int ci = i & 63, r = i >> 6, kw = r % 3, t = r / 3, tap = (2 - kp) * 3 + (2 - kw);
+#pragma unroll
+      for (int j = 0; j < 8; ++j) wv[j] = tile[j * 192 + kw * 64 + ci];
+      packed[(((ci >> 4) * G::NCH + tap * 2 + (T8 >> 2)) * 3 + t) * 64 + (T8 & 3) * 16 + (ci & 15)] = split_slot(wv, t);
+      return;
+    }
+    default: {
+      if (i >= 576) return;
+      using G = X9Geom<X9_CONV3>;
+      const int r = i & 7, u = (i >> 3) % 24, t = i / 192, k0 = kp * 192 + 8 * u, co = T8 * 8 + r;
+#pragma unroll
+      for (int j = 0; j < 8; ++j) wv[j] = tile[r * 192 + 8 * u + j];
+      packed[(((co >> 4) * G::NCH + (k0 >> 5)) * 3 + t) * 64 + ((k0 >> 3) & 3) * 16 + (co & 15)] = split_slot(wv, t);
+      return;
+    }
+  }
+}
+constexpr int kTilePackMax = 576;
+
+__global__ __launch_bounds__(kOptThreads) void k_adam_pack(AdamPackArgs pk, OptArgs a, const double *__restrict__ part,
+                                                          int nparts, ScalarArgs sa, float w1, float beta2, float w2,
+                                                          float eps) {
+  __shared__ __attribute__((aligned(16))) float tile[kPackTileMax];
+  const int64_t b = blockIdx.x;
+  if (b >= pk.blocks) {
+    const OptSeg &sg = a.seg[seg_of(a, b - pk.blocks)];
+    adam_wg<false>(sg, (b - pk.blocks - sg.blk0) * kAdamChunk, part, nparts, sa, w1, beta2, w2, eps, false, nullptr);
+    return;
+  }
+  int s = 0;
+  while (s + 1 < pk.nseg && b >= pk.seg[s + 1].blk0) ++s;
+  const int K = pk.K[s], L = pk.L[s], parts = K / L;
+  const int T = (int)(b - pk.seg[s].blk0), T8 = T / parts, kp = T - T8 * parts;
+  const OptSeg &sg = pk.seg[s];
+  adam_wg<true>(sg, 0, part, nparts, sa, w1, beta2, w2, eps, b == 0, tile,
+                AdamTile{(int64_t)T8 * kPackTileCo * K + kp * L, K, L, kPackTileCo * L / 4});
+  __syncthreads();
+  for (int l = 0; l < pk.n; ++l) {
+    if (pk.seg_of[l] != s) continue;
+    for (int i = threadIdx.x; i < kTilePackMax; i += kOptThreads) tile_pack(pk.geom[l], T8, kp, i, tile, pk.packed[l]);
   }
 }
 
@@ -315,6 +410,100 @@
   return RTH_OK;
 }
 
+static int adam_pack_launch(const char *who, const rth_param_tensor *tensors, int32_t n_tensors, double lr, double beta1,
+                            double beta2, double eps, double max_norm, int64_t *step_dev, void *workspace_dev,
+                            float *total_norm_out, int nparts, bool sqsum, int32_t n_jobs, const rth_conv_shape *shapes,
+                            const int32_t *job_tensor, float *const *packed, hipStream_t s) {
+  RTH_REQUIRE(n_jobs >= 0 && n_jobs <= kPackMax && (n_jobs == 0 || (shapes && job_tensor && packed)),
+              "%s: bad pack jobs", who);
+  if (n_jobs == 0)
+    return adam_launch(who, tensors, n_tensors, lr, beta1, beta2, eps, max_norm, step_dev, workspace_dev,
+                       total_norm_out, nparts, sqsum, s);
+  RTH_REQUIRE(tensors && n_tensors >= 1 && n_tensors <= RTH_MAX_PARAM_TENSORS, "%s: %d tensors not in [1, %d]", who,
+              n_tensors, RTH_MAX_PARAM_TENSORS);
+  AdamPackArgs pk{};
+  int seg_tensor[kAdamPackSegs];
+  for (int l = 0; l < n_jobs; ++l) {
+    rth_conv_shape fw = shapes[l];
+    int geom = -1;
+    if (fw.input & RTH_CONV_PACK_DGRAD) {
+      fw.input &= ~RTH_CONV_PACK_DGRAD;
+      geom = is_dgrad3_x9(&fw) ? kPackDgrad3 : (is_dgrad2_x9(&fw) ? kPackDgrad2 : -1);
+    } else {
+      ConvLaunch cl;
+      if (!find_conv(fw, &cl, &geom)) geom = -1;
+    }
+    RTH_REQUIRE(geom == 0 || geom == 2 || geom == 3 || geom == kPackDgrad3 || geom == kPackDgrad2,
+                "%s: pack job %d: geometry not written by the optimizer step", who, l);
+    const int ti = job_tensor[l];
+    RTH_REQUIRE(ti >= 0 && ti < n_tensors, "%s: pack job %d names tensor %d of %d", who, l, ti, n_tensors);
+    const int64_t K = (int64_t)fw.kh * fw.kw * fw.cin;
+    RTH_REQUIRE(tensors[ti].n == K * fw.cout && fw.cout % kPackTileCo == 0,
+                "%s: pack job %d: tensor %d has %lld elements, the geometry %lld", who, l, ti, (long long)tensors[ti].n,
+                (long long)(K * fw.cout));
+    RTH_REQUIRE(packed[l] && (reinterpret_cast<uintptr_t>(packed[l]) & 15) == 0, "%s: pack job %d buffer NULL or misaligned",
+                who, l);
+    int sgi = 0;
+    while (sgi < pk.nseg && seg_tensor[sgi] != ti) ++sgi;
+    if (sgi == pk.nseg) {
+      RTH_REQUIRE(pk.nseg < kAdamPackSegs, "%s: pack jobs on more than %d tensors", who, kAdamPackSegs);
+      const rth_param_tensor &t = tensors[ti];
+      RTH_REQUIRE(t.param && t.grad && t.exp_avg && t.exp_avg_sq, "%s: tensor %d incomplete", who, ti);
+      const uintptr_t al = reinterpret_cast<uintptr_t>(t.param) | reinterpret_cast<uintptr_t>(t.grad) |
+                           reinterpret_cast<uintptr_t>(t.exp_avg) | reinterpret_cast<uintptr_t>(t.exp_avg_sq);
+      RTH_REQUIRE((al & 15) == 0, "%s: tensor %d with pack jobs is not 16-byte aligned", who, ti);
+      seg_tensor[sgi] = ti;
+      pk.seg[sgi] = OptSeg{t.param, t.grad, t.exp_avg, t.exp_avg_sq, t.n, pk.blocks, 1};
+      pk.K[sgi] = (int)K;
+      pk.L[sgi] = geom == 0 ? 128 : fw.kw * fw.cin;
+      pk.blocks += fw.cout / kPackTileCo * (int)(K / pk.L[sgi]);
+      ++pk.nseg;
+    }
+    RTH_REQUIRE(pk.K[sgi] == K, "%s: pack job %d disagrees with tensor %d's other jobs", who, l, ti);
+    RTH_REQUIRE(K % pk.L[sgi] == 0 && pk.L[sgi] % 4 == 0 && kPackTileCo * pk.L[sgi] <= kPackTileMax &&
+                    kPackTileMax <= kAdamChunk,
+                "%s: pack job %d: no tile for this geometry", who, l);
+    pk.geom[l] = geom;
+    pk.seg_of[l] = sgi;
+    pk.packed[l] = reinterpret_cast<u32x4 *>(packed[l]);
+  }
+  pk.n = n_jobs;
+  AdamStep st{};
+  if (const int rc = adam_prepare(who, tensors, n_tensors, lr, beta1, beta2, max_norm, step_dev, workspace_dev,
+                                  total_norm_out, nparts, sqsum, s, &st))
+    return rc;
+  rth_param_tensor rest[RTH_MAX_PARAM_TENSORS];
+  int n_rest = 0;
+  for (int i = 0; i < n_tensors; ++i) {
+    bool tiled = false;
+    for (int k = 0; k < pk.nseg; ++k) tiled = tiled || seg_tensor[k] == i;
+    if (!tiled) rest[n_rest++] = tensors[i];
+  }
+  OptArgs ad{};
+  const int64_t ablocks = opt_segments(rest, n_rest, kAdamChunk, &ad);
+  hipLaunchKernelGGL(k_adam_pack, dim3((unsigned)(pk.blocks + ablocks)), dim3(kOptThreads), 0, s, pk, ad, st.part,
+                     st.nparts, st.sa, (float)(1.0 - beta1), (float)beta2, (float)(1.0 - beta2), (float)eps);
+  RTH_LAUNCHED();
+  return RTH_OK;
+}
+
+int rth_clip_adam_pack(const rth_param_tensor *tensors, int32_t n_tensors, double lr, double beta1, double beta2,
+                       double eps, double max_norm, int64_t *step_dev, void *workspace_dev, float *total_norm_out,
+                       int32_t n_jobs, const rth_conv_shape *shapes, const int32_t *job_tensor, float *const *packed,
+                       void *stream) {
+  return adam_pack_launch("rth_clip_adam_pack", tensors, n_tensors, lr, beta1, beta2, eps, max_norm, step_dev,
+                          workspace_dev, total_norm_out, 0, true, n_jobs, shapes, job_tensor, packed, as_stream(stream));
+}
+
+int rth_adam_prenormed_pack(const rth_param_tensor *tensors, int32_t n_tensors, double lr, double beta1, double beta2,
+                            double eps, double max_norm, int32_t nparts, int64_t *step_dev, void *workspace_dev,
+                            float *total_norm_out, int32_t n_jobs, const rth_conv_shape *shapes,
+                            const int32_t *job_tensor, float *const *packed, void *stream) {
+  return adam_pack_launch("rth_adam_prenormed_pack", tensors, n_tensors, lr, beta1, beta2, eps, max_norm, step_dev,
+                          workspace_dev, total_norm_out, nparts, false, n_jobs, shapes, job_tensor, packed,
+                          as_stream(stream));
+}
+
 static bool is_conv1_u8(const rth_conv_shape *s) {
   return s && s->input == RTH_CONV_U8_CHW && s->cin == 4 && s->hin == 84 && s->win == 84 && s->cout == 32 &&
          s->kh == 8 && s->kw == 8 && s->stride == 4;
diff --git a/reth_amd/csrc/optim.hip b/reth_amd/csrc/optim.hip
--- a/reth_amd/csrc/optim.hip
+++ b/reth_amd/csrc/optim.hip
@@ -1,33 +1,6 @@
 #include "optim.hpp"
 
 namespace rth {
-
-struct OptScalars {
-  float coef;
-  float step_size;
-  float bc2_sqrt;
-  float total_norm;
-};
-
-__device__ OptScalars opt_scalars(double acc, double *red, int clip, float max_norm, BiasCorr bc) {
-  const float total = (float)sqrt(block_sum(acc, red));
-  float coef = 1.0f;
-  if (clip) {
-    const float c = max_norm / radd(total, 1e-6f);
-    coef = c < 1.0f ? c : 1.0f;
-  }
-  return OptScalars{coef, bc.step_size, bc.bc2_sqrt, total};
-}
-
-struct ScalarArgs {
-  int clip;
-  float max_norm;
-  double lr, beta1, beta2;
-  int64_t *step;
-  OptScalars *out;
-  float *total_out;
-  BiasCorr *bc;
-};
 
 __global__ __launch_bounds__(kOptThreads) void k_grad_sqsum(OptArgs a, double *__restrict__ part, ScalarArgs sa) {
   grad_sqsum_wg(a, blockIdx.x, part, SqStep{sa.step, sa.bc, sa.lr, sa.beta1, sa.beta2});
@@ -35,92 +8,16 @@
 
 __global__ __launch_bounds__(kOptThreads) void k_adam(OptArgs a, const double *__restrict__ part, int nparts,
                                                      ScalarArgs sa, float w1, float beta2, float w2, float eps) {
-  __shared__ double red[kOptThreads / 64];
   const int64_t b = blockIdx.x;
   const OptSeg &sg = a.seg[seg_of(a, b)];
-  const int64_t base = (b - sg.blk0) * kAdamChunk;
-  double pacc = 0.0, pl[kPartLoads];
-#pragma unroll
-  for (int u = 0; u < kPartLoads; ++u) {
-    const int k = threadIdx.x + u * kOptThreads;
-    pl[u] = part[k < nparts ? k : nparts - 1];
-  }
-  const BiasCorr bc = *sa.bc;
-  auto sum_parts = [&]() __attribute__((always_inline)) {
-    __builtin_amdgcn_sched_barrier(0);
-#pragma unroll
-    for (int u = 0; u < kPartLoads; ++u) asm volatile("" : "+v"(pl[u]));
-#pragma unroll
-    for (int u = 0; u < kPartLoads; ++u)
-      if (threadIdx.x + u * kOptThreads < nparts) pacc = radd(pacc, pl[u]);
-    for (int k = threadIdx.x + kPartLoads * kOptThreads; k < nparts; k += kOptThreads) pacc = radd(pacc, part[k]);
-  };
-  __builtin_amdgcn_sched_barrier(0);
-  float4 gv[kAdamV], mv[kAdamV], vv[kAdamV], pv[kAdamV];
-  if (sg.vec) {
-    const __amdgpu_buffer_rsrc_t rg = seg_rsrc(sg.grad, sg.n), rm = seg_rsrc(sg.m, sg.n), rv = seg_rsrc(sg.v, sg.n),
-                                 rp = seg_rsrc(sg.param, sg.n);
-#pragma unroll
-    for (int k = 0; k < kAdamV; ++k) {
-      const int64_t e = base + 4 * (k * kOptThreads + threadIdx.x);
-      gv[k] = ld4b(rg, e);
-      mv[k] = ld4b(rm, e);
-      vv[k] = ld4b(rv, e);
-      pv[k] = ld4b(rp, e);
-    }
-    sum_parts();
-  } else {
-#pragma unroll
-    for (int k = 0; k < kAdamV; ++k) {
-      const int64_t e = base + 4 * (k * kOptThreads + threadIdx.x);
-      gv[k] = ld4(sg.grad, e, sg.n, 0);
-      mv[k] = ld4(sg.m, e, sg.n, 0);
-      vv[k] = ld4(sg.v, e, sg.n, 0);
-      pv[k] = ld4(sg.param, e, sg.n, 0);
-    }
-    sum_parts();
-  }
-  const OptScalars sc = opt_scalars(pacc, red, sa.clip, sa.max_norm, bc);
-  if (b == 0 && threadIdx.x == 0) {
-    *sa.out = sc;
-    if (sa.total_out) *sa.total_out = sc.total_norm;
-  }
-  const int clip = sa.clip;
-  const float coef = sc.coef, step_size = sc.step_size, bc2_sqrt = sc.bc2_sqrt;
-  auto adam1 = [&](float g, float &m, float &v, float &p) {
-    if (clip) g = rmul(g, coef);
-    m = radd(m, rmul(w1, rsub(g, m)));
-    v = radd(rmul(v, beta2), rmul(rmul(w2, g), g));
-    const float denom = radd(sqrtf(v) / bc2_sqrt, eps);
-    p = radd(p, rmul(-step_size, m) / denom);
-  };
-#pragma unroll
-  for (int k = 0; k < kAdamV; ++k) {
-    const int64_t e = base + 4 * (k * kOptThreads + threadIdx.x);
-    if (e >= sg.n) break;
-    adam1(gv[k].x, mv[k].x, vv[k].x, pv[k].x);
-    adam1(gv[k].y, mv[k].y, vv[k].y, pv[k].y);
-    adam1(gv[k].z, mv[k].z, vv[k].z, pv[k].z);
-    adam1(gv[k].w, mv[k].w, vv[k].w, pv[k].w);
-    st4(sg.param, e, sg.n, sg.vec, pv[k]);
-    st4(sg.m, e, sg.n, sg.vec, mv[k]);
-    st4(sg.v, e, sg.n, sg.vec, vv[k]);
-  }
+  adam_wg<false>(sg, (b - sg.blk0) * kAdamChunk, part, nparts, sa, w1, beta2, w2, eps, b == 0, nullptr);
 }
-
-}
-
-using namespace rth;
-
-extern "C" {
-
-int64_t rth_clip_adam_workspace(void) { return (int64_t)kMaxPartials * 8 + 64; }
 
 constexpr int64_t kMaxTensorElems = (int64_t)1 << 29;
 
-static int adam_launch(const char *who, const rth_param_tensor *tensors, int32_t n_tensors, double lr, double beta1,
-                       double beta2, double eps, double max_norm, int64_t *step_dev, void *workspace_dev,
-                       float *total_norm_out, int nparts, bool sqsum, hipStream_t s) {
+int adam_prepare(const char *who, const rth_param_tensor *tensors, int32_t n_tensors, double lr, double beta1,
+                 double beta2, double max_norm, int64_t *step_dev, void *workspace_dev, float *total_norm_out,
+                 int nparts, bool sqsum, hipStream_t s, AdamStep *out) {
   RTH_REQUIRE(tensors && step_dev && workspace_dev, "%s: NULL argument", who);
   RTH_REQUIRE(n_tensors >= 1 && n_tensors <= RTH_MAX_PARAM_TENSORS, "%s: %d tensors not in [1, %d]", who, n_tensors,
               RTH_MAX_PARAM_TENSORS);
@@ -130,9 +27,8 @@
     RTH_REQUIRE(tensors[i].n < kMaxTensorElems, "%s: tensor %d has %lld elements (fewer than 2^29 = %lld)", who, i,
                 (long long)tensors[i].n, (long long)kMaxTensorElems);
   }
-  OptArgs a{}, ad{};
+  OptArgs a{};
   const int64_t blocks = opt_segments(tensors, n_tensors, kOptChunk, &a);
-  const int64_t ablocks = opt_segments(tensors, n_tensors, kAdamChunk, &ad);
   if (sqsum) nparts = (int)(blocks < kMaxPartials ? blocks : kMaxPartials + 1);
   RTH_REQUIRE(nparts >= 1 && nparts <= kMaxPartials, "%s: %d norm partials (at most %d)", who, nparts, kMaxPartials);
   auto *part = static_cast<double *>(workspace_dev);
@@ -144,11 +40,32 @@
     hipLaunchKernelGGL(k_grad_sqsum, dim3((unsigned)blocks), dim3(kOptThreads), 0, s, a, part, sa);
     RTH_LAUNCHED();
   }
-  hipLaunchKernelGGL(k_adam, dim3((unsigned)ablocks), dim3(kOptThreads), 0, s, ad, part, nparts, sa,
+  *out = AdamStep{sa, part, nparts};
+  return RTH_OK;
+}
+
+int adam_launch(const char *who, const rth_param_tensor *tensors, int32_t n_tensors, double lr, double beta1,
+                double beta2, double eps, double max_norm, int64_t *step_dev, void *workspace_dev,
+                float *total_norm_out, int nparts, bool sqsum, hipStream_t s) {
+  AdamStep st{};
+  if (const int rc = adam_prepare(who, tensors, n_tensors, lr, beta1, beta2, max_norm, step_dev, workspace_dev,
+                                  total_norm_out, nparts, sqsum, s, &st))
+    return rc;
+  OptArgs ad{};
+  const int64_t ablocks = opt_segments(tensors, n_tensors, kAdamChunk, &ad);
+  hipLaunchKernelGGL(k_adam, dim3((unsigned)ablocks), dim3(kOptThreads), 0, s, ad, st.part, st.nparts, st.sa,
                      (float)(1.0 - beta1), (float)beta2, (float)(1.0 - beta2), (float)eps);
   RTH_LAUNCHED();
   return RTH_OK;
 }
+
+}
+
+using namespace rth;
+
+extern "C" {
+
+int64_t rth_clip_adam_workspace(void) { return (int64_t)kMaxPartials * 8 + 64; }
 
 int rth_clip_adam(const rth_param_tensor *tensors, int32_t n_tensors, double lr, double beta1, double beta2,
                   double eps, double max_norm, int64_t *step_dev, void *workspace_dev, float *total_norm_out,
diff --git a/reth_amd/csrc/optim.hpp b/reth_amd/csrc/optim.hpp
--- a/reth_amd/csrc/optim.hpp
+++ b/reth_amd/csrc/optim.hpp
@@ -89,6 +89,134 @@
 }
 
 
+struct OptScalars {
+  float coef;
+  float step_size;
+  float bc2_sqrt;
+  float total_norm;
+};
+
+__device__ __forceinline__ OptScalars opt_scalars(double acc, double *red, int clip, float max_norm, BiasCorr bc) {
+  const float total = (float)sqrt(block_sum(acc, red));
+  float coef = 1.0f;
+  if (clip) {
+    const float c = max_norm / radd(total, 1e-6f);
+    coef = c < 1.0f ? c : 1.0f;
+  }
+  return OptScalars{coef, bc.step_size, bc.bc2_sqrt, total};
+}
+
+struct ScalarArgs {
+  int clip;
+  float max_norm;
+  double lr, beta1, beta2;
+  int64_t *step;
+  OptScalars *out;
+  float *total_out;
+  BiasCorr *bc;
+};
+
+struct AdamTile {
+  int64_t origin;
+  int K, L, groups;
+};
+
+template <bool TILE>
+__device__ __forceinline__ void adam_wg(const OptSeg &sg, const int64_t base, const double *__restrict__ part,
+                                        int nparts, const ScalarArgs &sa, float w1, float beta2, float w2, float eps,
+                                        bool first, float *tile, const AdamTile tm = AdamTile{}) {
+  auto elem = [&](int k) __attribute__((always_inline)) -> int64_t {
+    if constexpr (TILE) {
+      const int g = k * kOptThreads + threadIdx.x, r = 4 * g / tm.L, c = 4 * g - r * tm.L;
+      return g < tm.groups ? tm.origin + (int64_t)r * tm.K + c : sg.n;
+    } else {
+      return base + 4 * (k * kOptThreads + threadIdx.x);
+    }
+  };
+  __shared__ double red[kOptThreads / 64];
+  double pacc = 0.0, pl[kPartLoads];
+#pragma unroll
+  for (int u = 0; u < kPartLoads; ++u) {
+    const int k = threadIdx.x + u * kOptThreads;
+    pl[u] = part[k < nparts ? k : nparts - 1];
+  }
+  const BiasCorr bc = *sa.bc;
+  auto sum_parts = [&]() __attribute__((always_inline)) {
+    __builtin_amdgcn_sched_barrier(0);
+#pragma unroll
+    for (int u = 0; u < kPartLoads; ++u) asm volatile("" : "+v"(pl[u]));
+#pragma unroll
+    for (int u = 0; u < kPartLoads; ++u)
+      if (threadIdx.x + u * kOptThreads < nparts) pacc = radd(pacc, pl[u]);
+    for (int k = threadIdx.x + kPartLoads * kOptThreads; k < nparts; k += kOptThreads) pacc = radd(pacc, part[k]);
+  };
+  __builtin_amdgcn_sched_barrier(0);
+  float4 gv[kAdamV], mv[kAdamV], vv[kAdamV], pv[kAdamV];
+  if (sg.vec) {
+    const __amdgpu_buffer_rsrc_t rg = seg_rsrc(sg.grad, sg.n), rm = seg_rsrc(sg.m, sg.n), rv = seg_rsrc(sg.v, sg.n),
+                                 rp = seg_rsrc(sg.param, sg.n);
+#pragma unroll
+    for (int k = 0; k < kAdamV; ++k) {
+      const int64_t e = elem(k);
+      gv[k] = ld4b(rg, e);
+      mv[k] = ld4b(rm, e);
+      vv[k] = ld4b(rv, e);
+      pv[k] = ld4b(rp, e);
+    }
+    sum_parts();
+  } else {
+#pragma unroll
+    for (int k = 0; k < kAdamV; ++k) {
+      const int64_t e = elem(k);
+      gv[k] = ld4(sg.grad, e, sg.n, 0);
+      mv[k] = ld4(sg.m, e, sg.n, 0);
+      vv[k] = ld4(sg.v, e, sg.n, 0);
+      pv[k] = ld4(sg.param, e, sg.n, 0);
+    }
+    sum_parts();
+  }
+  const OptScalars sc = opt_scalars(pacc, red, sa.clip, sa.max_norm, bc);
+  if (first && threadIdx.x == 0) {
+    *sa.out = sc;
+    if (sa.total_out) *sa.total_out = sc.total_norm;
+  }
+  const int clip = sa.clip;
+  const float coef = sc.coef, step_size = sc.step_size, bc2_sqrt = sc.bc2_sqrt;
+  auto adam1 = [&](float g, float &m, float &v, float &p) {
+    if (clip) g = rmul(g, coef);
+    m = radd(m, rmul(w1, rsub(g, m)));
+    v = radd(rmul(v, beta2), rmul(rmul(w2, g), g));
+    const float denom = radd(sqrtf(v) / bc2_sqrt, eps);
+    p = radd(p, rmul(-step_size, m) / denom);
+  };
+#pragma unroll
+  for (int k = 0; k < kAdamV; ++k) {
+    const int64_t e = elem(k);
+    if (e >= sg.n) break;
+    adam1(gv[k].x, mv[k].x, vv[k].x, pv[k].x);
+    adam1(gv[k].y, mv[k].y, vv[k].y, pv[k].y);
+    adam1(gv[k].z, mv[k].z, vv[k].z, pv[k].z);
+    adam1(gv[k].w, mv[k].w, vv[k].w, pv[k].w);
+    st4(sg.param, e, sg.n, sg.vec, pv[k]);
+    st4(sg.m, e, sg.n, sg.vec, mv[k]);
+    st4(sg.v, e, sg.n, sg.vec, vv[k]);
+    if constexpr (TILE) *reinterpret_cast<float4 *>(tile + 4 * (k * kOptThreads + threadIdx.x)) = pv[k];
+  }
+}
+
+struct AdamStep {
+  ScalarArgs sa;
+  const double *part;
+  int nparts;
+};
+int adam_prepare(const char *who, const rth_param_tensor *tensors, int32_t n_tensors, double lr, double beta1,
+                 double beta2, double max_norm, int64_t *step_dev, void *workspace_dev, float *total_norm_out,
+                 int nparts, bool sqsum, hipStream_t s, AdamStep *out);
+int adam_launch(const char *who, const rth_param_tensor *tensors, int32_t n_tensors, double lr, double beta1,
+                double beta2, double eps, double max_norm, int64_t *step_dev, void *workspace_dev,
+                float *total_norm_out, int nparts, bool sqsum, hipStream_t s);
+
+
 struct SqStep {
   int64_t *step;
   BiasCorr *bc;
diff --git a/reth_amd/fused_learner.py b/reth_amd/fused_learner.py
--- a/reth_amd/fused_learner.py
+++ b/reth_amd/fused_learner.py
@@ -16,6 +16,7 @@
 DGRAD_MASK = True
 DGRAD_NCHW = os.environ.get("RTH_DGRAD_NCHW", "1") != "0"
 NORM_IN_BACKWARD = True
+ADAM_PACK = os.environ.get("RTH_ADAM_PACK", "0") == "1"
 
 
 def eligible(net, s0, s1):
@@ -31,6 +32,35 @@
         return False
     shapes = net._torso_shapes(tuple(s0.shape[1:]), s0.dtype == torch.uint8)
     return all(sh is not None for _, sh in shapes)
+
+
+def learner_packs(solver, net, shapes, u8, device, create=True):
+    from .optim import ClipAdam
+
+    if not (ADAM_PACK and u8 and DGRAD_PREPACK and isinstance(solver.optimizer, ClipAdam)):
+        return None
+    if any(sh is None for sh in shapes) or shapes[0].input != _lib.CONV_U8_CHW:
+        return None
+    convs = net._convs()
+    if not all(c.weight.is_contiguous(memory_format=torch.channels_last) for c in convs):
+        return None
+    layers = tuple(li for li in sorted(HIP_DGRAD)
+                   if li < len(shapes) and _lib.lib().rth_conv_dgrad_workspace(ctypes.byref(shapes[li])) > 0)
+    store = net.__dict__.setdefault("_workspaces", {})
+    key = (device, "learner_packs", tuple((sh.input, sh.cin, sh.hin, sh.cout) for sh in shapes), layers)
+    packs = store.get(key)
+    if packs is None and create:
+        packs = store[key] = model.LearnerPacks(net, shapes, layers, device)
+    return packs
+
+
+def refresh_packs(net):
+    n = 0
+    for key, packs in net.__dict__.get("_workspaces", {}).items():
+        if len(key) > 1 and key[1] == "learner_packs" and not packs.current():
+            packs.pack()
+            n += 1
+    return n
 
 
 def _pair(s0, s1):
@@ -67,16 +97,23 @@
         hp = net._head_params()
         fc2p = net._fc2_ptrs(hp)[0]
         dgp, extra = {}, []
-        if DGRAD_PREPACK:
-            for li in HIP_DGRAD:
-                sh = shapes[li] if li < len(shapes) else None
-                if sh is None or _lib.lib().rth_conv_dgrad_workspace(ctypes.byref(sh)) <= 0:
-                    continue
-                dgp[li] = conv_workspace(net, "dgrad", _lib.lib().rth_conv_dgrad_workspace, sh, x.device)
-                flagged = _lib.ConvShape(sh.input | _lib.CONV_PACK_DGRAD, sh.cin, sh.hin, sh.win, sh.cout, sh.kh, sh.kw,
-                                         sh.stride)
-                extra.append((flagged, _nhwc(convs[li].weight.detach()).data_ptr(), dgp[li].data_ptr()))
-        packed = net.pack_convs(u8=u8, extra=extra)
+        packs = learner_packs(solver, net, shapes, u8, x.device)
+        if packs is not None:
+            dgp, packed = packs.dgrad, packs.packed
+            if not packs.current():
+                packs.pack()
+            solver.optimizer.pack_with_step(packs)
+        else:
+            if DGRAD_PREPACK:
+                for li in HIP_DGRAD:
+                    sh = shapes[li] if li < len(shapes) else None
+                    if sh is None or _lib.lib().rth_conv_dgrad_workspace(ctypes.byref(sh)) <= 0:
+                        continue
+                    dgp[li] = conv_workspace(net, "dgrad", _lib.lib().rth_conv_dgrad_workspace, sh, x.device)
+                    flagged = _lib.ConvShape(sh.input | _lib.CONV_PACK_DGRAD, sh.cin, sh.hin, sh.win, sh.cout, sh.kh,
+                                             sh.kw, sh.stride)
+                    extra.append((flagged, _nhwc(convs[li].weight.detach()).data_ptr(), dgp[li].data_ptr()))
+            packed = net.pack_convs(u8=u8, extra=extra)
         st = stream_ptr()
         ys, h = [], x
         probed = []
diff --git a/reth_amd/model.py b/reth_amd/model.py
--- a/reth_amd/model.py
+++ b/reth_amd/model.py
@@ -33,6 +33,51 @@
 def conv_workspace(owner, kind, sizer, shape, device):
     return workspace(owner, device, kind, (shape.input, shape.cin, shape.hin, shape.cout),
                      lambda: sizer(ctypes.byref(shape)))
+
+
+class LearnerPacks:
+
+    def __init__(self, net, shapes, dgrad_layers, device):
+        self.convs = net._convs()
+        self.packed = [torch.empty(lib().rth_conv_packed_bytes(ctypes.byref(sh)) // 4, dtype=torch.float32,
+                                   device=device) for sh in shapes]
+        self.dgrad = {li: conv_workspace(net, "dgrad", lib().rth_conv_dgrad_workspace, shapes[li], device)
+                      for li in dgrad_layers}
+        self.jobs = [(sh, c.weight, buf) for sh, c, buf in zip(shapes, self.convs, self.packed)]
+        for li, buf in self.dgrad.items():
+            sh = shapes[li]
+            flagged = ConvShape(sh.input | _lib.CONV_PACK_DGRAD, sh.cin, sh.hin, sh.win, sh.cout, sh.kh, sh.kw, sh.stride)
+            self.jobs.append((flagged, self.convs[li].weight, buf))
+        self.stamp = None
+        self.launches = 0
+
+    def _now(self):
+        return tuple((c.weight._version, c.weight.data_ptr()) for c in self.convs)
+
+    def current(self):
+        return self.stamp is not None and self.stamp == self._now()
+
+    def invalidate(self):
+        self.stamp = None
+
+    def written(self):
+        if not torch.cuda.is_current_stream_capturing():
+            self.stamp = self._now()
+
+    @torch.no_grad()
+    def pack(self):
+        n, keep = len(self.jobs), []
+        ws = []
+        for _, p, _ in self.jobs:
+            w = p.detach()
+            if not w.is_contiguous(memory_format=torch.channels_last):
+                w = w.contiguous(memory_format=torch.channels_last)
+                keep.append(w)
+            ws.append(w.data_ptr())
+        call("rth_conv_pack_many", n, (ConvShape * n)(*[sh for sh, _, _ in self.jobs]), (c_vp * n)(*ws),
+             (c_vp * n)(*[buf.data_ptr() for _, _, buf in self.jobs]), stream_ptr())
+        self.launches += 1
+        self.written()
 
 
 def _copy_without(net, memo, skip):
diff --git a/reth_amd/optim.py b/reth_amd/optim.py
--- a/reth_amd/optim.py
+++ b/reth_amd/optim.py
@@ -31,6 +31,7 @@
         self._ws = torch.zeros(_lib.lib().rth_clip_adam_workspace(), dtype=torch.uint8, device=dev)
         self.total_norm = torch.zeros(1, dtype=torch.float32, device=dev)
         self._prenormed = None
+        self._packs = self._packs_seen = None
         for p in ps:
             st = self.state[p]
             st["exp_avg"] = torch.zeros_like(p)
@@ -43,10 +44,11 @@
         g = self.param_groups[0]
         beta1, beta2 = g["betas"]
         mn = self.max_norm if max_norm is None else max_norm
-        tensors = []
+        tensors, index = [], {}
         for p in g["params"]:
             if p.grad is None:
                 continue
+            index[id(p)] = len(tensors)
             gr = p.grad
             if gr.stride() != p.stride():
                 gr = torch.empty_like(p).copy_(gr)
@@ -57,15 +59,40 @@
             return loss
         arr = (ParamTensor * len(tensors))(*tensors)
         nparts, self._prenormed = self._prenormed, None
+        packs, self._packs = self._packs, None
+        jobs = self._pack_jobs(packs, index) if packs is not None else None
+        if self._packs_seen is not None and (jobs is None or packs is not self._packs_seen):
+            self._packs_seen.invalidate()
+        head = (ctypes.cast(arr, _lib.c_vp), len(tensors), float(g["lr"]), float(beta1), float(beta2), float(g["eps"]),
+                -1.0 if mn is None or mn < 0 else float(mn))
+        tail = (ptr(self._step), ptr(self._ws), ptr(self.total_norm))
+        if jobs is not None:
+            self._packs_seen = packs
+            if nparts is not None:
+                call("rth_adam_prenormed_pack", *head, nparts, *tail, *jobs, stream_ptr())
+            else:
+                call("rth_clip_adam_pack", *head, *tail, *jobs, stream_ptr())
+            packs.written()
+            return loss
         if nparts is not None:
-            call("rth_adam_prenormed", ctypes.cast(arr, _lib.c_vp), len(tensors), float(g["lr"]), float(beta1),
-                 float(beta2), float(g["eps"]), -1.0 if mn is None or mn < 0 else float(mn), nparts, ptr(self._step),
-                 ptr(self._ws), ptr(self.total_norm), stream_ptr())
+            call("rth_adam_prenormed", *head, nparts, *tail, stream_ptr())
             return loss
-        call("rth_clip_adam", ctypes.cast(arr, _lib.c_vp), len(tensors), float(g["lr"]), float(beta1), float(beta2),
-             float(g["eps"]), -1.0 if mn is None or mn < 0 else float(mn), ptr(self._step), ptr(self._ws),
-             ptr(self.total_norm), stream_ptr())
+        call("rth_clip_adam", *head, *tail, stream_ptr())
         return loss
+
+    def pack_with_step(self, packs):
+        self._packs = packs
+
+    @staticmethod
+    def _pack_jobs(packs, index):
+        jobs = packs.jobs
+        if not jobs or any(id(p) not in index or not p.is_contiguous(memory_format=torch.channels_last)
+                           for _, p, _ in jobs):
+            return None
+        n = len(jobs)
+        return (n, (_lib.ConvShape * n)(*[sh for sh, _, _ in jobs]),
+                (_lib.c_i32 * n)(*[index[id(p)] for _, p, _ in jobs]),
+                (_lib.c_vp * n)(*[buf.data_ptr() for _, _, buf in jobs]))
 
     def norm_tensors(self, grads):
         ts = [ParamTensor(gr.data_ptr(), gr.data_ptr(), gr.data_ptr(), gr.data_ptr(), gr.numel()) for gr in grads]
@@ -78,9 +105,10 @@
 
     def step_launch(self, max_norm=None):
         nparts, self._prenormed = self._prenormed, None
+        packs, self._packs = self._packs, None
 
         def launch():
-            self._prenormed = nparts
+            self._prenormed, self._packs = nparts, packs
             self.step(max_norm=max_norm)
 
         return launch
diff --git a/reth_amd/solver.py b/reth_amd/solver.py
--- a/reth_amd/solver.py
+++ b/reth_amd/solver.py
@@ -308,6 +308,9 @@
         self.last_loss = loss.detach()
         return td_abs
 
+    def refresh_learner_packs(self):
+        return fused_learner.refresh_packs(self.q_network)
+
     def apply_grads(self, probe=None):
         if isinstance(self.optimizer, ClipAdam):
             if probe is not None:
```
